# RMDLO/trackdlo

Measured on AMD Instinct MI355X. Metric: EM iterations/sec at N=50k cloud pts, M=50 nodes, higher is better.
Workload: dtype f32; 1 GPU; C2: 1 frame(s) per GPU, N=50000 points, M=50 nodes, 50 EM iterations per cpd_lle call, tol=0, trackdlo.launch parameters, fp32 E-step + fp64 M-step; whole calls (prune + sort + setup + loop + read-back), sorted-cloud reuse OFF, calls alternate between 2 resident (cloud, Y0) pairs; frames_per_gpu=1, parallelism=frames sharded, 1 rank(s), no data-path collective

## Files before the change

trackdlo_amd/csrc/tdlo_api.cpp:

```cpp
#include "../../include/trackdlo_hip.h"
#include "tdlo_internal.h"
#include "tdlo_host.h"
#include "tdlo_image.h"
#include "tdlo_rccl.h"

#include <algorithm>
#include <limits>
#include <chrono>
#include <cmath>
#include <cstdio>
#include <cstdlib>
#include <cstring>
#include <condition_variable>
#include <functional>
#include <mutex>
#include <string>
#include <thread>
#include <vector>

using namespace tdlo;

namespace {

#define TDLO_RET(x) do { hipError_t e_ = (x); if (e_ != hipSuccess) return e_; } while (0)
// ... 68 lines not shown
    }
    void loop(int idx) {
        (void)hipSetDevice(device);
        int seen = 0;
        for (;;) {
            std::function<int(int)> f;
            {
                std::unique_lock<std::mutex> lk(m);
                cv.wait(lk, [&] { return stop || gen != seen; });
                if (stop) return;
                seen = gen; f = job;
            }
            const int rc = f(idx);
            {
                std::lock_guard<std::mutex> lk(m);
                if (rc && !first_err) first_err = rc;
                if (--pending == 0) cv_done.notify_one();
            }
        }
    }
    int run(const std::function<int(int)> &f) {
        {
            std::lock_guard<std::mutex> lk(m);
            job = f; pending = (int)th.size(); first_err = 0; ++gen;
        }
        cv.notify_all();
        const int rc0 = f(0);
        std::unique_lock<std::mutex> lk(m);
        cv_done.wait(lk, [&] { return pending == 0; });
        return rc0 ? rc0 : first_err;
    }
    ~EnqueuePool() {
        { std::lock_guard<std::mutex> lk(m); stop = true; }
        cv.notify_all();
        for (auto &t : th) t.join();
    }
};

struct tdlo_ctx {
    int device = 0;
    hipStream_t stream = nullptr;
    double *xfer = nullptr;
    size_t xfer_doubles = 0;
    hipStream_t stream2[kBatchStreams - 1] = {};
    hipEvent_t evx[kBatchStreams] = {}, evj[kBatchStreams] = {};
    hipEvent_t ev[6] = {nullptr, nullptr, nullptr, nullptr, nullptr, nullptr};
    tdlo_config cfg{};
    std::vector<Slot> slots;
    std::vector<FrameDev> fh;
    FrameDev *fd = nullptr;
    double *pin = nullptr;
    double *reg_ws = nullptr;
    size_t reg_ws_cap = 0;
    void *cloud_ws = nullptr;
    size_t cloud_ws_cap = 0;
    void *cloud_fws = nullptr;
    size_t cloud_fws_cap = 0;
    bool cloud_fused_first = true;
    unsigned long long *cloud_res = nullptr;
    unsigned cloud_epoch = 0;
    char *img_pin = nullptr;
    size_t img_pin_cap = 0;
    int img_pin_rows = 0, img_pin_cols = 0;
    bool cloud_fused_on = !(getenv("TDLO_CLOUD_FUSED") && atoi(getenv("TDLO_CLOUD_FUSED")) == 0);
    bool cloud_team_on = !(getenv("TDLO_CLOUD_TEAM") && atoi(getenv("TDLO_CLOUD_TEAM")) == 0);
    unsigned long long *vis_state = nullptr, *vis_res = nullptr;
    unsigned vis_epoch = 0;
    bool vis_armed = false;
    double *vis_nodes_pin = nullptr;
    long long cloud_vis_rides = 0;
    long long vis_route[2] = {0, 0};
    long long cloud_route[2] = {0, 0};
    char *col_pin = nullptr;
    size_t col_pin_cap = 0;
    int col_pin_rows = 0, col_pin_cols = 0;
    void *col_dev = nullptr;
    size_t col_dev_cap = 0;
    bool colour_fused_on = !(getenv("TDLO_COLOUR_FUSED") && atoi(getenv("TDLO_COLOUR_FUSED")) == 0);
    long long colour_route[2] = {0, 0};
    const unsigned char *last_colour = nullptr, *last_occluder = nullptr;
    const void *view_img[4] = {nullptr, nullptr, nullptr, nullptr};
    int view_rows = 0, view_cols = 0;
    int last_col_rows = 0, last_col_cols = 0;
    char *res_pin = nullptr;
    size_t res_pin_cap = 0;
    int res_pin_rows = 0, res_pin_cols = 0;
    void *res_dev = nullptr;
    size_t res_dev_cap = 0;
    char *rnd_pin = nullptr, *rnd_dev = nullptr;
    bool render_inplace = !(getenv("TDLO_RENDER_INPLACE") && atoi(getenv("TDLO_RENDER_INPLACE")) == 0);
    long long render_route[2] = {0, 0};
    size_t pin_doubles = 0;
    std::string err;
    int last_F = 0;
    bool lle_batch_dense = false;
    bool lle_dense_once = false;
    long long band_retries = 0;
    long long route_count[6] = {0, 0, 0, 0, 0, 0};
    bool fuse_on = true;
    int fuse_force_timeout = getenv("TDLO_FUSE_FORCE_TIMEOUT") ? atoi(getenv("TDLO_FUSE_FORCE_TIMEOUT")) : 0;
    bool sort_reuse = !(getenv("TDLO_REUSE_SORT") && atoi(getenv("TDLO_REUSE_SORT")) == 0);
    double *mbox = nullptr;
    size_t mbox_doubles = 0;
    unsigned mbox_epoch = 0;
    bool direct_in = !(getenv("TDLO_DIRECT_UPLOAD") && atoi(getenv("TDLO_DIRECT_UPLOAD")) == 0);
    double *late_buf = nullptr;
    size_t late_doubles = 0;
    bool late_on = !(getenv("TDLO_LATE_PRIORS") && atoi(getenv("TDLO_LATE_PRIORS")) == 0);
    bool mbox_on = !(getenv("TDLO_HOST_MAILBOX") && atoi(getenv("TDLO_HOST_MAILBOX")) == 0);
    struct PairNext {
        int state = 0;
        int slot = 0, M = 0, n_vis = 0;
        double sigma2 = 0;
        tdlo_params p{};
        std::vector<double> Y;
        FrameDev f{};
        size_t up = 0;
        bool has_sums = false;
        bool ahead = false;
        bool cloud_in_pin = false;
        int spec = 0;
        unsigned spec_epoch = 0;
    } pair;
    double *pin2 = nullptr;
    size_t pin2_doubles = 0;
    bool pair_on = !(getenv("TDLO_PAIR_SETUP") && atoi(getenv("TDLO_PAIR_SETUP")) == 0);
    Slot twin;
    bool twin_busy = false;
    bool ahead_on = !(getenv("TDLO_AHEAD") && atoi(getenv("TDLO_AHEAD")) == 0);
    double *cloud_pin = nullptr;
    size_t cloud_pin_doubles = 0;
    int cloud_pending = -1;
    bool cloud_direct_on = !(getenv("TDLO_DIRECT_CLOUD") && atoi(getenv("TDLO_DIRECT_CLOUD")) == 0);
    bool view_inplace = !(getenv("TDLO_VIEW_INPLACE") && atoi(getenv("TDLO_VIEW_INPLACE")) == 0);
    long long view_route[2] = {0, 0};
    long long voxel_view_calls = 0;
    hipEvent_t ev_view = nullptr;
    int iter_hint = 0, iter_hint_next = 0;
    bool iter_hint_on = !(getenv("TDLO_ITER_HINT") && atoi(getenv("TDLO_ITER_HINT")) == 0);
    bool lle_next_on = !(getenv("TDLO_LLE_NEXT") && atoi(getenv("TDLO_LLE_NEXT")) == 0);
    bool spec_force_timeout = getenv("TDLO_SPEC_FORCE_TIMEOUT") && atoi(getenv("TDLO_SPEC_FORCE_TIMEOUT")) != 0;
    bool spec_on = !(getenv("TDLO_SPEC_MSTEP") && atoi(getenv("TDLO_SPEC_MSTEP")) == 0);
    bool pair_sums_on = !(getenv("TDLO_PAIR_SUMS") && atoi(getenv("TDLO_PAIR_SUMS")) == 0);
    int estep2_mode = getenv("TDLO_ESTEP2") ? atoi(getenv("TDLO_ESTEP2")) : -1;
    int estep2_rows = (getenv("TDLO_ESTEP2_ROWS") && atoi(getenv("TDLO_ESTEP2_ROWS")) == 16) ? 16 : 8;
    int estep2_blocks = getenv("TDLO_ESTEP2_BLOCKS") ? atoi(getenv("TDLO_ESTEP2_BLOCKS")) : 0;
    bool xch_self = getenv("TDLO_XCH_SELF") && atoi(getenv("TDLO_XCH_SELF")) != 0;
    bool boost_off_once = false;
    long long boost_retries = 0;
    bool test_boost_fail = getenv("TDLO_TEST_BOOST_FAIL") && atoi(getenv("TDLO_TEST_BOOST_FAIL")) != 0;
    int estep_wide_min = getenv("TDLO_ESTEP_WIDE") ? (atoi(getenv("TDLO_ESTEP_WIDE")) > 0 ? atoi(getenv("TDLO_ESTEP_WIDE")) : (1 << 30)) : kEstepWideMin;
    int fused_iter_mode = getenv("TDLO_FUSED_ITER") ? (atoi(getenv("TDLO_FUSED_ITER")) != 0 ? 1 : 0) : -1;
    long long fused_calls = 0;
    long long estep2_frames = 0;
    bool timing = false;
    EnqueuePool *pool = nullptr;
    int split_active = 0;
    double *xch_dmin = nullptr;
    double *xch_sums = nullptr;
    double *split_buf = nullptr;
    size_t split_buf_doubles = 0;
    void *own_comm = nullptr;
    unsigned long long *xch_own = nullptr;
    size_t xch_own_words = 0;
    int xch_rank = 0, xch_nranks = 0, xch_mcap = 0, xch_cap_ranks = 0;
    unsigned long long *xch_peer[kMaxXchRanks] = {};
    std::vector<void *> xch_opened;
    unsigned xch_calls = 0;
};

namespace {

struct HostProf {
    static constexpr int kN = 16;
    const char *name[kN] = {"set_cloud call", "guide nodes", "prepare_frame #1", "enqueue prologue #1", "enqueue iteration #1", "wait #1", "results #1",
                            "traverse + priors", "prepare_frame #2", "enqueue prologue #2", "enqueue iteration #2", "wait #2", "results #2", "between registrations", "", ""};
    double us[kN] = {};
    long n[kN] = {};
    bool on = getenv("TDLO_TRACK_PROFILE") && atoi(getenv("TDLO_TRACK_PROFILE")) != 0;
    int base = 0;
    std::chrono::steady_clock::time_point t0;
    void start() { if (on) t0 = std::chrono::steady_clock::now(); }
    void mark(int id) {
        if (!on) return;
        const auto t1 = std::chrono::steady_clock::now();
        us[id] += std::chrono::duration<double, std::micro>(t1 - t0).count(); ++n[id];
        t0 = t1;
    }
    void report() {
        if (!on) return;
        double tot = 0;
        for (int i = 0; i < kN; ++i) if (n[i]) tot += us[i] / (double)n[i];
        fprintf(stderr, "trackdlo_hip host profile (us per call of the phase; sum %.1f):\n", tot);
        for (int i = 0; i < kN; ++i) if (n[i]) fprintf(stderr, "  %-24s %8.2f  x %ld\n", name[i], us[i] / (double)n[i], n[i]);
    }
};
HostProf g_prof;

int fail(tdlo_ctx *c, int code, const std::string &msg) {
    if (c) c->err = msg;
    if (code == TDLO_E_HIP) (void)hipGetLastError();
    return code;
}

#define HIPCHK(c, call)                                                                        \
    do {                                                                                       \
        hipError_t e_ = (call);                                                                \
        if (e_ != hipSuccess)                                                                  \
            return fail((c), TDLO_E_HIP, std::string(#call) + ": " + hipGetErrorString(e_));   \
    } while (0)

hipError_t wait_stream(hipStream_t s) {
    static const int spin_us = getenv("TDLO_SPIN_US") ? atoi(getenv("TDLO_SPIN_US")) : 0;
    if (spin_us > 0) {
        const auto t0 = std::chrono::steady_clock::now();
        for (;;) {
            const hipError_t e = hipStreamQuery(s);
            if (e != hipErrorNotReady) return e;
            if (std::chrono::duration<double, std::micro>(std::chrono::steady_clock::now() - t0).count() > spin_us) break;
        }
    }
    return hipStreamSynchronize(s);
}

hipError_t drain_for_realloc(tdlo_ctx *c) {
    const hipError_t e = hipStreamSynchronize(c->stream);
    if (e != hipSuccess) return e;
    if (c->stream2[0]) return hipStreamSynchronize(c->stream2[0]);
    return hipSuccess;
}

enum class Staging {
    Pinned,
    PinnedZeroed,
    DeviceZeroed
};
static int grow_staging(tdlo_ctx *c, double *&buf, size_t &have, size_t doubles, Staging kind) {
    if (doubles <= have) return 0;
    const bool dev = kind == Staging::DeviceZeroed;
    HIPCHK(c, dev ? hipStreamSynchronize(c->stream) : drain_for_realloc(c));
    if (buf) { if (dev) hipFree(buf); else hipHostFree(buf); }
    buf = nullptr; have = 0;
    if (dev) {
        HIPCHK(c, hipMalloc((void **)&buf, doubles * sizeof(double)));
        HIPCHK(c, hipMemsetAsync(buf, 0, doubles * sizeof(double), c->stream));
    } else {
        HIPCHK(c, hipHostMalloc((void **)&buf, doubles * sizeof(double), hipHostMallocDefault));
        if (kind == Staging::PinnedZeroed) std::memset(buf, 0, doubles * sizeof(double));
    }
    have = doubles;
    return 0;
}
int ensure_pin(tdlo_ctx *c, size_t doubles) { return grow_staging(c, c->pin, c->pin_doubles, doubles, Staging::Pinned); }
int ensure_pin2(tdlo_ctx *c, size_t doubles) { return grow_staging(c, c->pin2, c->pin2_doubles, doubles, Staging::Pinned); }
int ensure_late(tdlo_ctx *c, size_t doubles) { return grow_staging(c, c->late_buf, c->late_doubles, doubles, Staging::PinnedZeroed); }
int ensure_mbox(tdlo_ctx *c, size_t doubles) { return grow_staging(c, c->mbox, c->mbox_doubles, doubles, Staging::PinnedZeroed); }
int ensure_cloud_pin(tdlo_ctx *c, size_t doubles) {
    if (doubles <= c->cloud_pin_doubles) return 0;
    return grow_staging(c, c->cloud_pin, c->cloud_pin_doubles, (doubles + 4095) & ~(size_t)4095, Staging::Pinned);
}
int ensure_xfer(tdlo_ctx *c, size_t doubles) { return grow_staging(c, c->xfer, c->xfer_doubles, doubles, Staging::DeviceZeroed); }

int mbox_wait(tdlo_ctx *c, hipStream_t stream, unsigned epoch, int min_it, bool need_done, unsigned long long *word) {
    const unsigned long long *w = (const unsigned long long *)(c->mbox + c->mbox_doubles - 2);
    auto t_chk = std::chrono::steady_clock::now();
    for (unsigned spins = 1;; ++spins) {
        const unsigned long long v = __atomic_load_n(w, __ATOMIC_ACQUIRE);
        if ((unsigned)(v >> 32) == epoch) {
            const bool done = (v >> 31) & 1u;
            if (done || (!need_done && (int)(v & 0x7fffffffu) >= min_it)) { *word = v; return 0; }
        }
        if ((spins & 255u) == 0) {
            const auto now = std::chrono::steady_clock::now();
            if (std::chrono::duration<double, std::micro>(now - t_chk).count() > 500.0) {
                t_chk = now;
                const hipError_t e = hipStreamQuery(stream);
                if (e == hipSuccess) {
                    const unsigned long long v2 = __atomic_load_n(w, __ATOMIC_ACQUIRE);
                    if ((unsigned)(v2 >> 32) == epoch && (((v2 >> 31) & 1u) || (!need_done && (int)(v2 & 0x7fffffffu) >= min_it))) { *word = v2; return 0; }
                    return 1;
                }
                if (e != hipErrorNotReady) return fail(c, TDLO_E_HIP, std::string("stream: ") + hipGetErrorString(e));
            }
        }
#if defined(__x86_64__)
        __builtin_ia32_pause();
#endif
    }
}

int ensure_points(tdlo_ctx *c, Slot &s, int n) {
    if (n <= s.cap_points) return 0;
    HIPCHK(c, drain_for_realloc(c));
    if (s.Xraw) hipFree(s.Xraw);
    if (s.Xs) hipFree(s.Xs);
    if (s.bucket) hipFree(s.bucket);
    if (s.blksum) hipFree(s.blksum);
    s.Xraw = nullptr; s.Xs = nullptr; s.bucket = nullptr; s.blksum = nullptr;
    s.cap_points = 0; s.N0 = 0;
    const size_t cap = ((size_t)n + 1023) & ~(size_t)1023;
    const size_t nb = cap / kBlock + 1;
    HIPCHK(c, hipMalloc((void **)&s.Xraw, 3 * cap * sizeof(double)));
    HIPCHK(c, hipMalloc((void **)&s.Xs, 3 * cap * sizeof(double)));
    HIPCHK(c, hipMalloc((void **)&s.bucket, cap * sizeof(unsigned short)));
    HIPCHK(c, hipMalloc((void **)&s.blksum, (nb + 2) * sizeof(double)));
    s.cap_points = (int)cap;
// ... 258 lines not shown
            HIPCHK(c, hipMalloc((void **)&s.hist, 2 * need * sizeof(int)));
            s.hist_ints = need;
        }
    }
    f.Xraw = s.Xraw; f.Xs = s.Xs; f.bucket = s.bucket; f.hist = s.hist; f.hist_off = s.hist + (size_t)f.nprune_blocks * M; f.blksum = s.blksum;
    f.keep = s.blksum + (size_t)s.cap_points / kBlock + 1;
    f.reuse_sorted = (c->sort_reuse && s.sorted_valid && s.sorted_prec == p->precision && s.sorted_Y.size() == 3 * (size_t)M &&
                      std::memcmp(s.sorted_Y.data(), Y, sizeof(double) * 3 * M) == 0) ? 1 : 0;
    f.Yin = blk + nc.Yin; f.ctr = blk + nc.ctr; f.Y = blk + nc.Y; f.Y0 = blk + nc.Y0; f.nodes = blk + nc.nodes;
    f.coord = blk + nc.coord; f.G = blk + nc.G; f.chain = blk + nc.chain; f.H = blk + nc.H; f.Hb = blk + nc.Hb; f.HG = blk + nc.HG; f.HY0 = blk + nc.HY0;
    f.aJ = blk + nc.aJ; f.aYd = blk + nc.aYd; f.dminbits = (unsigned long long *)(blk + nc.dmin);
    f.acc = (long long *)(blk + nc.acc);
    f.band = blk + nc.band;
    {
        int ln = 0; while (((long long)1 << ln) < (long long)s.N0 + 1) ++ln;
        double len = 0;
        for (int i = 0; i + 1 < M; ++i) { double d2 = 0; for (int d = 0; d < 3; ++d) { const double e = Y[d * M + i + 1] - Y[d * M + i]; d2 += e * e; } len += std::sqrt(d2); }
        int ld = 0; while (std::ldexp(1.0, ld) < 2.0 * (len + 0.2) && ld < 20) ++ld;
        static const int sh_coarser = getenv("TDLO_ACC_COARSER") ? atoi(getenv("TDLO_ACC_COARSER")) : 0;
        const int shP = std::min(60 - ln, 44) - sh_coarser;
        f.acc_sh[0] = shP; f.acc_sh[1] = shP - ld; f.acc_sh[2] = shP - 2 * ld;
        {
            static const int only = getenv("TDLO_ACC_COARSER_ONLY") ? atoi(getenv("TDLO_ACC_COARSER_ONLY")) : -1;
            if (only >= 0) for (int k = 0; k < 3; ++k) if (k != only) f.acc_sh[k] += sh_coarser;
        }
        const int lshare = std::min(51, 67 - std::max(ln, 6)), lpoint = std::min(51, 61 - ln);
        f.acc_lim[0] = std::ldexp(1.0, lshare - f.acc_sh[0]); f.acc_lim[1] = std::ldexp(1.0, lshare - f.acc_sh[1]); f.acc_lim[2] = std::ldexp(1.0, lpoint - f.acc_sh[2]);
    }
    f.acc_boost_off = c->boost_off_once ? 1 : (c->test_boost_fail ? -1 : 0);
    f.estep_wide_min = c->estep_wide_min;
    if (estep2_eligible(c, f) && (c->estep2_mode == 1 || nbatch >= kEstep2MinWaves)) estep2_geometry(c, f, false);
    choose_acc_rows(c, f, false);
    f.sums = blk + nc.sums; f.Ascr = blk + nc.Ascr; f.Yout = blk + nc.Yout; f.dbg = (unsigned long long *)(blk + nc.dbg);
    f.sync = s.sync;
    f.st = (IterState *)(blk + nc.st);
    if (hb_resident) f.Hb = s.hb_next;
    return 0;
}

hipError_t zero_accumulators(const std::vector<FrameDev> &fh, int F, hipStream_t s) {
    for (int i = 0; i < F; ++i) {
        const hipError_t e = hipMemsetAsync(fh[i].acc, 0, sizeof(long long) * 2 * kAccRows * (4 * (size_t)fh[i].M + 2), s);
        if (e != hipSuccess) return e;
    }
    return hipSuccess;
}

size_t upload_doubles(const NodeCarve &nc, const tdlo_params *p, bool band) { return p->include_lle ? (band ? nc.H : nc.upload) : nc.Hb; }

void fill_stats(tdlo_stats *st, const IterState &is) {
    st->iters = is.it; st->converged = is.converged; st->n_kept = is.N; st->status = is.status; st->sigma2 = is.sigma2;
    st->mstep_retries = is.retries;
}

typedef std::function<int(const double *&, int &)> LatePriors;

static unsigned next_mbox_epoch(tdlo_ctx *c) {
    unsigned e = ++c->mbox_epoch;
    if (e == 0) e = ++c->mbox_epoch;
    return e;
}

static FrameDev spec_mstep_descriptor(tdlo_ctx *c, const tdlo_ctx::PairNext &pn, unsigned epoch, const IterState *spec_prev, double *lle_next) {
    FrameDev fs = pn.f;
    fs.reuse_sorted = 1; fs.has_priors = 1;
    fs.late_aJ = c->late_buf; fs.late_aYd = c->late_buf + pn.M;
    fs.host_out = c->mbox; fs.host_prog = (unsigned long long *)(c->mbox + c->mbox_doubles - 2); fs.host_epoch = epoch;
    fs.host_report_it = (pn.p.tol <= 0.0 || pn.p.max_iter <= 2 * kChunkIters) ? 0 : std::max(1, std::min(std::min(c->iter_hint_next, kIterHintMax), pn.p.max_iter));
    fs.spec_flag = spec_flag_word(c); fs.spec_prev = spec_prev; fs.spec_epoch = epoch;
    if (lle_next) fs.lle_next = lle_next;
    return fs;
}

static int launch_ahead(tdlo_ctx *c) {
    tdlo_ctx::PairNext &pn = c->pair;
    const int M = pn.M;
    const int N0 = c->slots[pn.slot].N0;
    const NodeCarve nc(M);
    if (!pn.cloud_in_pin || N0 <= 0 || pn.p.include_lle || pn.p.max_iter <= 0 || M > kChainLdsMaxNodes) return 0;
    if (c->late_doubles < 4 * (size_t)M + 2 || c->mbox_doubles < nc.readback + 4 || c->cloud_pin_doubles < 3 * (size_t)N0) return 0;
    if (!c->stream2[0]) HIPCHK(c, hipStreamCreateWithFlags(&c->stream2[0], hipStreamNonBlocking));
    hipStream_t sb = c->stream2[0];
    Slot &tw = c->twin;
    const size_t need_hist = (size_t)((N0 + kBlock - 1) / kBlock) * M;
    const bool grow = N0 > tw.cap_points || M > tw.cap_nodes || need_hist > tw.hist_ints || nc.upload + 2 > c->pin2_doubles;
    if (grow || c->twin_busy) HIPCHK(c, hipStreamSynchronize(sb));
    c->twin_busy = false;
    int rc;
    if ((rc = ensure_points(c, tw, N0))) return rc;
    tw.N0 = N0; tw.sorted_valid = false;
    if ((rc = ensure_pin2(c, nc.upload + 2))) return rc;
    FrameDev &f = pn.f;
    if ((rc = prepare_frame(c, -1, pn.Y.data(), M, pn.sigma2, &pn.p, nullptr, 0, nullptr, pn.n_vis, nullptr, c->pin2, f, false))) return rc;
    if (grow) HIPCHK(c, hipStreamSynchronize(c->stream));
    if (!f.wide_tile || f.mstep_dense || f.reuse_sorted || !c->fuse_on || !prologue_pair_ok(f)) return 0;
    pn.up = upload_doubles(nc, &pn.p, false);
    f.Xhost = c->cloud_pin;
    std::memcpy(c->pin2 + nc.fdev, &f, sizeof(FrameDev));
    const unsigned fep = next_fuse_epoch(c, tw);
    c->twin_busy = true;
    HIPCHK(c, launch_prologue_direct(&f, c->pin2, tw.nodeblk, (int)pn.up, (int)nc.Yin, fep, sb));
    f.Xhost = nullptr;
    f.late_mstep = 1;
    const FrameDev *fdb = (const FrameDev *)(tw.nodeblk + nc.fdev);
    if (f.vis_branch) HIPCHK(c, launch_estep_only(fdb, &f, 1, 1, sb));
    HIPCHK(c, launch_estep_only(fdb, &f, 1, 0, sb));
    const unsigned e2 = next_mbox_epoch(c);
    const FrameDev fs = spec_mstep_descriptor(c, pn, e2, nullptr, nullptr);
    HIPCHK(c, launch_mstep_chain(fdb, &fs, 1, 0, fs.precision == TDLO_PREC_F64, sb));
    pn.has_sums = false; pn.spec = 1; pn.spec_epoch = e2; pn.ahead = true; pn.state = 2;
    return 0;
}

static int chunk_iters(int chunk, int left) { return std::min(chunk < 2 ? 1 : (chunk == 2 ? 2 : kChunkIters), left); }

static IterState readback_state(const double *blocks, size_t stride, const NodeCarve &nc, int i) {
    IterState is;
    std::memcpy(&is, blocks + (size_t)i * stride + (nc.st - nc.Yout), sizeof is);
    return is;
}
static bool every_frame_done(const double *blocks, size_t stride, const NodeCarve &nc, int F) {
    for (int i = 0; i < F; ++i) if (readback_state(blocks, stride, nc, i).done == 0) return false;
    return true;
}
static bool any_frame_ended_with(int status, const double *blocks, size_t stride, const NodeCarve &nc, int F) {
    for (int i = 0; i < F; ++i) if (readback_state(blocks, stride, nc, i).status == status) return true;
    return false;
}

int run_frames(tdlo_ctx *c, int F, const int *slots, double *Y, int M, double *sigma2, const tdlo_params *p,
               const double *priors, int K, const int *vis, int n_vis, const double *H_override, tdlo_stats *stats,
               const LatePriors *late = nullptr);

struct SpecGuard {
    tdlo_ctx *c; unsigned epoch = 0; bool live = false;
    void release(bool go) { if (live) { spec_release(c, epoch, go); live = false; } }
    ~SpecGuard() { release(false); }
};

struct FramesCall {
    tdlo_ctx *const c; const int F; const int *const slots; double *const Y; const int M; double *const sigma2; const tdlo_params *const p;
    const double *const priors; const int K; const int *const vis; const int n_vis; const double *const H_override; tdlo_stats *const stats;
    const LatePriors *const late;
    const int iter_hint;
    const bool timing;
    const NodeCarve nc;
    const bool merged;
    size_t up, ustride;
    const size_t fdd;
    bool paired = false;
    bool ahead = false;
    bool use_mbox = false;
    bool fused_mode = false;
    bool late_async = false;
    bool lle_next = false;
    hipStream_t s = nullptr;
    hipStream_t gs[kBatchStreams] = {};
    int goff[kBatchStreams + 1] = {};
    int NS = 1;
    bool forked = false;
    int enqueued = 0;
    bool sums_first = false;
    bool ahead_first = false;
    bool spec_released = false;
    unsigned epoch = 0;
    bool have_readback = false;
    const FrameDev *fdp = nullptr;
    double *nodeblk_used = nullptr;
    SpecGuard sg;

    FramesCall(tdlo_ctx *c_, int F_, const int *slots_, double *Y_, int M_, double *sigma2_, const tdlo_params *p_, const double *priors_, int K_,
               const int *vis_, int n_vis_, const double *H_override_, tdlo_stats *stats_, const LatePriors *late_, int iter_hint_)
        : c(c_), F(F_), slots(slots_), Y(Y_), M(M_), sigma2(sigma2_), p(p_), priors(priors_), K(K_), vis(vis_), n_vis(n_vis_), H_override(H_override_),
          stats(stats_), late(late_), iter_hint(iter_hint_), timing(c_->timing), nc(M_), merged(F_ > 1),
          up(upload_doubles(nc, p_, p_->include_lle && mstep_band_enabled() && !c_->lle_dense_once)), ustride(merged ? up : nc.upload),
          fdd(((size_t)F_ * sizeof(FrameDev) + 15) / 16 * 2), sg{c_} {}

    Slot &slot0() const { return c->slots[slots[0]]; }
    size_t rstride() const { return merged ? nc.readback : nc.upload; }
    bool fixed_count() const { return p->tol <= 0.0 || p->max_iter <= 2 * kChunkIters; }

    int size_staging();
    void recognise_pair();
    int stage_frames();
    int choose_batch_kernels();
    int choose_routes();
    int open_mailbox();
    int upload_and_prologue();
    int stage_late_priors();
    int fork_streams();
    void choose_loop();
    int drive_fixed();
    int drive_mailbox();
    int drive_polled();
    int read_back();
    bool repeat(int *rc);
    int results_out(std::chrono::steady_clock::time_point t_host0);

    FrameDev fused_copy(int k) const;
    hipError_t iterate(int n);
    hipError_t join();
    int mbox_done(int min_it, bool need_done, bool *done);
    int take_mbox(bool events_recorded);
    int launch_paired_mstep_ahead();
};

int FramesCall::size_staging() {
    int rc = ensure_pin(c, (size_t)F * std::max(nc.upload, nc.readback + 2) + fdd + 2 * (size_t)F * std::max(nc.readback, (sizeof(IterState) + 7) / 8) + 4);
    if (rc) return rc;
    if (merged) rc = ensure_xfer(c, (size_t)F * (upload_doubles(nc, p, false) + nc.readback) + fdd);
    return rc;
}

void FramesCall::recognise_pair() {
    if (late && c->pair.state == 2) {
        const tdlo_ctx::PairNext &pn = c->pair;
        const Slot &sl = slot0();
        const bool same = F == 1 && !priors && !H_override && pn.slot == slots[0] && pn.M == M && pn.n_vis == n_vis && pn.sigma2 == sigma2[0] && same_params(pn.p, *p) &&
                          std::memcmp(pn.Y.data(), Y, sizeof(double) * 3 * M) == 0 && pn.f.wide_tile != 0;
        if (pn.ahead) paired = ahead = same && c->stream2[0] != nullptr;
        else paired = same && sl.sorted_valid && sl.sorted_prec == p->precision &&
                      sl.sorted_Y.size() == 3 * (size_t)M && std::memcmp(sl.sorted_Y.data(), Y, sizeof(double) * 3 * M) == 0;
        c->pair.state = 0; c->pair.ahead = false;
    }
    if (late && c->pair.spec) { sg.epoch = c->pair.spec_epoch; sg.live = true; c->pair.spec = 0; }
    if (!paired) sg.release(false);
    c->fh.assign(F, FrameDev{});
    if (paired) {
        c->fh[0] = c->pair.f; c->fh[0].reuse_sorted = 1; up = c->pair.up;
        if (ahead) ++c->route_count[4];
        else { ++c->route_count[0]; if (c->pair.has_sums) ++c->route_count[1]; }
    }
}

int FramesCall::stage_frames() {
    for (int pass = 0; pass < 2 && !paired; ++pass) {
        for (int i = 0; i < F; ++i) {
            const int rc = prepare_frame(c, slots[i], Y + (size_t)i * 3 * M, M, sigma2[i], p, priors, K, vis, n_vis, H_override,
                                         c->pin + (size_t)i * ustride, c->fh[i], false, !merged);
            if (rc) return rc;
            if (merged) {
                FrameDev &f = c->fh[i];
                f.wide_tile = 0;
                if (c->cfg.estep_blocks <= 0 && f.nblkE >= 64) f.nblkE = (f.nblkE + 1) / 2;
                double *bu = c->xfer + (size_t)i * up, *br = c->xfer + (size_t)F * up + fdd + (size_t)i * nc.readback;
                f.Yin = bu + nc.Yin; f.aJ = bu + nc.aJ; f.aYd = bu + nc.aYd;
                if (p->include_lle) { f.Hb = bu + nc.Hb; f.H = bu + nc.H; }
                f.Yout = br; f.st = (IterState *)(br + (nc.st - nc.Yout));
            }
        }
        if (merged) { const int rc = choose_batch_kernels(); if (rc) return rc; }
        if (!p->include_lle) break;
        bool all_band = true;
        for (int i = 0; i < F; ++i) all_band = all_band && c->fh[i].lle_band;
        if (all_band) break;
        if (!merged) { up = upload_doubles(nc, p, false); break; }
        if (pass == 0) { c->lle_batch_dense = true; up = upload_doubles(nc, p, false); ustride = up; }
    }
    c->lle_batch_dense = false;
    return 0;
}

int FramesCall::choose_batch_kernels() {
    long long waves = 0;
    bool elig = true;
    for (int i = 0; i < F; ++i) { waves += (c->fh[i].N0 + 63) / 64; elig = elig && estep2_eligible(c, c->fh[i]); }
    const bool two = elig && (c->estep2_mode == 1 || waves >= kEstep2MinWaves);
    for (int i = 0; i < F; ++i) if (two) estep2_geometry(c, c->fh[i], true);
    for (int i = 0; i < F; ++i) choose_acc_rows(c, c->fh[i], true);
    {
        static const int env = getenv("TDLO_ACC_ROWS") ? atoi(getenv("TDLO_ACC_ROWS")) : 0;
        bool small = env == 0 && !p->include_lle;
        for (int i = 0; i < F; ++i) small = small && c->fh[i].nblkE <= 64 && !c->fh[i].mstep_dense && c->fh[i].M <= kChunk;
        if (small) for (int i = 0; i < F; ++i) c->fh[i].acc_rows = 2;
    }
    if (!two) for (int i = 0; i < F; ++i) if (c->fh[i].estep2) return fail(c, TDLO_E_INVALID, "internal: a batch's frames disagree about the E-step kernel");
    return 0;
}

int FramesCall::choose_routes() {
    if (!merged && !paired && p->include_lle && c->fh[0].lle_band && slot0().hb_next != nullptr && c->fh[0].Hb == slot0().hb_next)
        { up = nc.Hb; ++c->route_count[3]; }
    lle_next = late != nullptr && !merged && !ahead && c->lle_next_on && !p->include_lle && !c->fh[0].mstep_dense && M <= 256 && p->max_iter > 0 &&
               slot0().hb_next_cap >= M;
    if (lle_next) { c->fh[0].lle_next = slot0().hb_next; slot0().hb_next_valid = false; }
    late_async = late != nullptr && c->fh[0].wide_tile != 0 && (c->late_on || paired);
    if (late && !late_async) {
        const double *lp = nullptr; int lk = 0;
        int rc;
        if ((rc = (*late)(lp, lk))) return rc;
        if ((rc = stage_priors(c, c->pin + nc.aJ, c->pin + nc.aYd, Y, M, lp, lk, p->alpha))) return rc;
        c->fh[0].has_priors = lk > 0 ? 1 : 0;
    }
    g_prof.mark(g_prof.base + 2);
    {
        bool all_reuse = true;
        for (int i = 0; i < F; ++i) all_reuse = all_reuse && c->fh[i].reuse_sorted;
        if (!all_reuse) for (int i = 0; i < F; ++i) c->fh[i].reuse_sorted = 0;
    }
    return 0;
}

int FramesCall::open_mailbox() {
    use_mbox = !merged && c->mbox_on && p->max_iter > 0 &&
               ((!p->include_lle && !c->fh[0].mstep_dense) || (p->include_lle && c->fh[0].lle_band));
    if (!use_mbox) { sg.release(false); return 0; }
    const int rc = ensure_mbox(c, nc.readback + 4);
    if (rc) return rc;
    epoch = sg.live ? sg.epoch : next_mbox_epoch(c);
    c->fh[0].host_out = c->mbox; c->fh[0].host_prog = (unsigned long long *)(c->mbox + c->mbox_doubles - 2); c->fh[0].host_epoch = epoch;
    return 0;
}

int FramesCall::upload_and_prologue() {
    int rc;
    s = ahead ? c->stream2[0] : c->stream;
    if (timing) HIPCHK(c, hipEventRecord(c->ev[0], s));
    if (merged) {
        std::memcpy(c->pin + (size_t)F * up, c->fh.data(), sizeof(FrameDev) * F);
        HIPCHK(c, hipMemcpyAsync(c->xfer, c->pin, ((size_t)F * up + fdd) * sizeof(double), hipMemcpyHostToDevice, s));
        fdp = (const FrameDev *)(c->xfer + (size_t)F * up);
    } else {
        if (!paired) std::memcpy(c->pin + nc.fdev, c->fh.data(), sizeof(FrameDev));
        nodeblk_used = ahead ? c->twin.nodeblk : (paired ? slot0().nodeblk2 : slot0().nodeblk);
        fdp = (const FrameDev *)(nodeblk_used + nc.fdev);
    }
    if (c->cloud_pending >= 0) {
        const bool fused = !merged && !paired && c->direct_in && c->fuse_on && c->cloud_pending == slots[0] && !c->fh[0].reuse_sorted && prologue_pair_ok(c->fh[0]);
        if (fused) { c->fh[0].Xhost = c->cloud_pin; c->cloud_pending = -1; }
        else if ((rc = flush_pending_cloud(c))) return rc;
    }
    if (paired) {
    } else if (!merged && c->direct_in && (c->fuse_on || c->fh[0].reuse_sorted) && prologue_direct_ok(c->fh[0])) {
        Slot &sl = slot0();
        const unsigned fep = c->fh[0].reuse_sorted ? 0u : next_fuse_epoch(c, sl);
        tdlo_ctx::PairNext &pn = c->pair;
        const FrameDev *f2 = nullptr;
        if (pn.state == 1) {
            pn.state = 0;
            if (!late && !c->fh[0].reuse_sorted && prologue_pair_ok(c->fh[0]) && pn.slot == slots[0] && pn.M == M && !pn.p.include_lle) {
                const NodeCarve nc2(pn.M);
                if ((rc = ensure_pin2(c, nc2.upload + 2))) return rc;
                if ((rc = prepare_frame(c, pn.slot, pn.Y.data(), pn.M, pn.sigma2, &pn.p, nullptr, 0, nullptr, pn.n_vis, nullptr, c->pin2, pn.f, true))) return rc;
                if (pn.f.wide_tile && !pn.f.mstep_dense && !pn.f.vis_branch) {
                    pn.up = upload_doubles(nc2, &pn.p, false);
                    std::memcpy(c->pin2 + nc2.fdev, &pn.f, sizeof(FrameDev));
                    f2 = &pn.f;
                    pn.has_sums = p->include_lle && c->fh[0].lle_band && !c->fh[0].vis_branch && p->mu == pn.p.mu && p->precision == pn.p.precision &&
                                  sigma2[0] == pn.sigma2 && std::memcmp(Y, pn.Y.data(), sizeof(double) * 3 * M) == 0 && p->max_iter > 0 && c->pair_sums_on;
                    if (pn.has_sums) c->fh[0].pair_sums = sl.nodeblk2 + nc2.sums;
                }
            }
        }
        HIPCHK(c, launch_prologue_direct(c->fh.data(), c->pin, sl.nodeblk, (int)up, (int)nc.Yin, fep, s, f2, c->pin2, sl.nodeblk2, f2 ? (int)pn.up : 0));
        c->fh[0].Xhost = nullptr;
        if (f2) pn.state = 2;
    } else {
        if (!merged) HIPCHK(c, hipMemcpyAsync(slot0().nodeblk, c->pin, up * sizeof(double), hipMemcpyHostToDevice, s));
        HIPCHK(c, launch_prune_and_setup(fdp, c->fh.data(), F, s));
    }
    g_prof.mark(g_prof.base + 3);
    for (int i = 0; i < F; ++i) {
        Slot &sl = c->slots[slots[i]];
        if (!c->fh[i].reuse_sorted) { sl.sorted_Y.assign(Y + (size_t)i * 3 * M, Y + (size_t)(i + 1) * 3 * M); sl.sorted_prec = p->precision; sl.sorted_valid = true; }
    }
    return 0;
}

int FramesCall::stage_late_priors() {
    if (late_async) {
        const double *lp = nullptr; int lk = 0;
        int rc = (*late)(lp, lk);
        if (!rc) rc = ensure_late(c, 4 * (size_t)M);
        if (!rc) rc = stage_priors(c, c->late_buf, c->late_buf + M, Y, M, lp, lk, p->alpha);
        if (rc) { sg.release(false); (void)hipStreamSynchronize(s); return rc; }
        if (lk <= 0) sg.release(false);
        c->fh[0].has_priors = lk > 0 ? 1 : 0;
        c->fh[0].late_aJ = c->late_buf; c->fh[0].late_aYd = c->late_buf + M;
        g_prof.mark(7);
    }
    if (timing) HIPCHK(c, hipEventRecord(c->ev[1], s));
    return 0;
}

int FramesCall::fork_streams() {
    static const int ns_env = getenv("TDLO_BATCH_STREAMS") ? atoi(getenv("TDLO_BATCH_STREAMS")) : 0;
    NS = ns_env > 0 ? ns_env : (F >= 28 ? 3 : (F >= 16 ? 4 : (F >= 8 ? 2 : 1)));
    NS = std::max(1, std::min(std::min(NS, kBatchStreams), F));
    for (int g = 0; g <= NS; ++g) goff[g] = (int)(((long long)F * g) / NS);
    gs[0] = s;
    for (int g = 1; g < NS; ++g) {
        if (!c->stream2[g - 1]) HIPCHK(c, hipStreamCreateWithFlags(&c->stream2[g - 1], hipStreamNonBlocking));
        gs[g] = c->stream2[g - 1];
    }
    return 0;
}

void FramesCall::choose_loop() {
    sums_first = paired && !ahead && c->pair.has_sums;
    ahead_first = ahead;
    fused_mode = !merged && F == 1 && !paired && !ahead && late == nullptr && c->pair.state == 0 && use_mbox && !sums_first && !ahead_first &&
                 fused_iter_eligible(c, c->fh[0]);
    if (fused_mode) ++c->fused_calls;
}

FrameDev FramesCall::fused_copy(int k) const {
    FrameDev fc = c->fh[0];
    if (k & 1) { double *blk = nodeblk_used; fc.Yout = blk + nc.Yout2; fc.st = (IterState *)(blk + nc.st2); fc.Y = blk + nc.Y2; fc.nodes = blk + nc.nodes2; }
    return fc;
}

hipError_t FramesCall::iterate(int n) {
    for (int it = 0; it < n; ++it) {
        ++enqueued;
        if (fused_mode) {
            const int k = enqueued - 1;
            if (k == 0) TDLO_RET(launch_estep_only(fdp, c->fh.data(), 1, 0, s));
            if (k + 1 < p->max_iter) TDLO_RET(launch_iter_fused(fused_copy(k), fused_copy(k + 1), k, s));
            else TDLO_RET(launch_mstep_chain_close(fused_copy(k), k, s));
            continue;
        }
        if (sums_first || ahead_first) {
            const bool from_given = sums_first;
            sums_first = false; ahead_first = false;
            if (sg.live) { sg.release(!c->spec_force_timeout); spec_released = true; if (!ahead) ++c->route_count[2]; }
            else if (from_given) TDLO_RET(launch_mstep_chain(fdp, c->fh.data(), 1, 1, c->fh[0].precision == TDLO_PREC_F64, s));
            else {
                c->fh[0].late_mstep = 0;
                TDLO_RET(launch_iteration(fdp, c->fh.data(), 1, s));
            }
            c->fh[0].late_mstep = 0;
            continue;
        }
        for (int g = 0; g < NS; ++g) {
            const FrameDev *fdg = fdp + goff[g], *fhg = c->fh.data() + goff[g];
            const int Fg = goff[g + 1] - goff[g];
            if (NS > 1 && !forked && g + 1 < NS) {
                if (fhg[0].vis_branch) TDLO_RET(launch_estep_only(fdg, fhg, Fg, 1, gs[g]));
                TDLO_RET(launch_estep_only(fdg, fhg, Fg, 0, gs[g]));
                TDLO_RET(hipEventRecord(c->evx[g], gs[g]));
                TDLO_RET(hipStreamWaitEvent(gs[g + 1], c->evx[g], 0));
                TDLO_RET(launch_estep_only(fdg, fhg, Fg, 2, gs[g]));
            } else {
                TDLO_RET(launch_iteration(fdg, fhg, Fg, gs[g], enqueued - 1));
            }
        }
        forked = true;
    }
    return hipSuccess;
}

hipError_t FramesCall::join() {
    if (NS < 2 || !forked) return hipSuccess;
    for (int g = 1; g < NS; ++g) {
        TDLO_RET(hipEventRecord(c->evj[g - 1], gs[g]));
        TDLO_RET(hipStreamWaitEvent(s, c->evj[g - 1], 0));
    }
    return hipSuccess;
}

int FramesCall::mbox_done(int min_it, bool need_done, bool *done) {
    unsigned long long w = 0;
    int wr = mbox_wait(c, s, epoch, min_it, need_done, &w);
    if (wr == 1 && spec_released) {
        spec_released = false;
        IterState is;
        HIPCHK(c, hipMemcpy(&is, c->fh[0].st, sizeof is, hipMemcpyDeviceToHost));
        int have = is.it;
        if (!ahead && !is.done && have == 0 && enqueued > 0) { HIPCHK(c, launch_mstep_chain(fdp, c->fh.data(), 1, 1, c->fh[0].precision == TDLO_PREC_F64, s)); have = 1; }
        for (; !is.done && have < enqueued; ++have) HIPCHK(c, launch_iteration(fdp, c->fh.data(), 1, s));
        wr = mbox_wait(c, s, epoch, min_it, need_done, &w);
    }
    if (wr < 0) return wr;
    if (wr == 1) return fail(c, TDLO_E_HIP, "the stream drained, but the M-step did not report the state of the registration");
    *done = (w >> 31) & 1u;
    return 0;
}

int FramesCall::take_mbox(bool events_recorded) {
    std::memcpy(c->pin, c->mbox, nc.readback * sizeof(double));
    have_readback = true;
    if (timing) {
        if (!events_recorded) { HIPCHK(c, hipEventRecord(c->ev[2], s)); HIPCHK(c, hipEventRecord(c->ev[3], s)); }
        HIPCHK(c, hipEventSynchronize(c->ev[3]));
    }
    return 0;
}

int FramesCall::drive_fixed() {
    static const bool pool_on = !(getenv("TDLO_BATCH_THREADS") && atoi(getenv("TDLO_BATCH_THREADS")) == 0);
    int rc;
    if (NS > 1 && pool_on && p->max_iter >= 8) {
        HIPCHK(c, iterate(1));
        if (!c->pool) { c->pool = new EnqueuePool; c->pool->start(kBatchStreams - 1, c->device); }
        const int rest = p->max_iter - 1;
        const int prc = c->pool->run([&](int g) -> int {
            if (g >= NS) return 0;
            const FrameDev *fdg = fdp + goff[g], *fhg = c->fh.data() + goff[g];
            const int Fg = goff[g + 1] - goff[g];
            for (int it = 0; it < rest; ++it) { const hipError_t e = launch_iteration(fdg, fhg, Fg, gs[g], 1 + it); if (e != hipSuccess) return (int)e; }
            return 0;
        });
        if (prc) return fail(c, TDLO_E_HIP, std::string("batch enqueue: ") + hipGetErrorString((hipError_t)prc));
    } else {
        HIPCHK(c, iterate(p->max_iter));
    }
    if (use_mbox) {
        if (timing) { HIPCHK(c, hipEventRecord(c->ev[2], s)); HIPCHK(c, hipEventRecord(c->ev[3], s)); }
        bool done = false;
        if ((rc = mbox_done(0, true, &done))) return rc;
        if ((rc = take_mbox(true))) return rc;
    }
    return 0;
}

int FramesCall::launch_paired_mstep_ahead() {
    tdlo_ctx::PairNext &pn = c->pair;
    Slot &sl = slot0();
    const NodeCarve nc2(pn.M);
    const int rc = ensure_late(c, 4 * (size_t)pn.M + 2);
    if (rc) return rc;
    const unsigned e2 = next_mbox_epoch(c);
    const bool leaves_lle = c->lle_next_on && pn.M <= 256 && sl.hb_next_cap >= pn.M;
    const FrameDev fs = spec_mstep_descriptor(c, pn, e2, c->fh[0].st, leaves_lle ? sl.hb_next : nullptr);
    HIPCHK(c, launch_mstep_chain((const FrameDev *)(sl.nodeblk2 + nc2.fdev), &fs, 1, 1, fs.precision == TDLO_PREC_F64, s));
    pn.spec = 1; pn.spec_epoch = e2;
    return 0;
}

int FramesCall::drive_mailbox() {
    int rc;
    const int first = std::max(1, std::min(std::min(iter_hint, kIterHintMax), p->max_iter));
    c->fh[0].host_report_it = first;
    HIPCHK(c, iterate(first));
    if (!late && c->pair.state == 2 && c->pair.has_sums && c->spec_on && c->mbox_on && !timing && c->pair.p.max_iter > 0) {
        if ((rc = launch_paired_mstep_ahead())) return rc;
    } else if (!late && c->pair.state == 3) {
        c->pair.state = 0; c->pair.ahead = false;
        if (c->spec_on && c->mbox_on && !timing && c->pair.slot == slots[0] && (rc = launch_ahead(c))) { spec_abort(c); return rc; }
    }
    g_prof.mark(g_prof.base + 4);
    bool stop = false;
    if ((rc = mbox_done(first, false, &stop))) { spec_abort(c); return rc; }
    if (!stop && !c->pair.ahead) c->pair.spec = 0;
    g_prof.mark(g_prof.base + 5);
    int launched = first;
    for (int chunk = 0; launched < p->max_iter && !stop; ++chunk) {
        const int n = chunk_iters(chunk, p->max_iter - launched);
        c->fh[0].host_report_it = launched + n;
        HIPCHK(c, iterate(n));
        launched += n;
        if ((rc = mbox_done(launched - n, false, &stop))) return rc;
    }
    if (!stop && (rc = mbox_done(0, true, &stop))) return rc;
    return take_mbox(false);
}

int FramesCall::drive_polled() {
    IterState *flags = (IterState *)(c->pin + (size_t)F * nc.upload + fdd);
    double *fl_rb = c->pin + (size_t)F * nc.upload + fdd;
    const double *results_dev = merged ? c->xfer + (size_t)F * up + fdd : nodeblk_used + nc.Yout;
    HIPCHK(c, iterate(1));
    HIPCHK(c, join());
    if (timing) HIPCHK(c, hipEventRecord(c->ev[2], s));
    HIPCHK(c, hipMemcpyAsync(c->pin, results_dev, (size_t)F * nc.readback * sizeof(double), hipMemcpyDeviceToHost, s));
    if (timing) HIPCHK(c, hipEventRecord(c->ev[3], s));
    HIPCHK(c, wait_stream(s));
    have_readback = every_frame_done(c->pin, rstride(), nc, F);
    int launched = 1;
    bool stop = have_readback;
    for (int chunk = 0; launched < p->max_iter && !stop; ++chunk) {
// ... 1750 lines not shown
        double tot = 0;
        for (int r = -3; r < reps; ++r) {
            if (fh[0].vis_branch) HIPCHK(c, launch_estep_only(c->fd, fh.data(), F, 1, s));
            HIPCHK(c, launch_estep_only(c->fd, fh.data(), F, 0, s));
            if (kind == 4) HIPCHK(c, launch_estep_only(c->fd, fh.data(), F, 3, s));
            if (r >= 0) HIPCHK(c, hipEventRecord(evs[2 * r], s));
            HIPCHK(c, launch_estep_only(c->fd, fh.data(), F, kind, s));
            if (r >= 0) HIPCHK(c, hipEventRecord(evs[2 * r + 1], s));
            if (kind == 3) HIPCHK(c, launch_estep_only(c->fd, fh.data(), F, 4, s));
        }
        HIPCHK(c, hipStreamSynchronize(s));
        for (int r = 0; r < reps; ++r) { float ms = 0; hipEventElapsedTime(&ms, evs[2 * r], evs[2 * r + 1]); tot += ms; }
        for (auto &e : evs) hipEventDestroy(e);
        if (avg_us) *avg_us = (float)(tot * 1000.0 / reps);
    } else {
    for (int w = 0; w < 3; ++w) HIPCHK(c, launch_estep_only(c->fd, fh.data(), F, kind, s));
    HIPCHK(c, hipEventRecord(c->ev[0], s));
    for (int r = 0; r < reps; ++r) HIPCHK(c, launch_estep_only(c->fd, fh.data(), F, kind, s));
    HIPCHK(c, hipEventRecord(c->ev[1], s));
    HIPCHK(c, hipStreamSynchronize(s));
    float ms = 0;
    hipEventElapsedTime(&ms, c->ev[0], c->ev[1]);
    if (avg_us) *avg_us = ms * 1000.0f / (float)reps;
    }
    }
    HIPCHK(c, zero_accumulators(fh, F, s));
    for (int i = 0; i < F; ++i) {
        std::memcpy(c->pin + i * 16, &saved[i], sizeof(IterState));
        HIPCHK(c, hipMemcpyAsync(c->fh[i].st, c->pin + i * 16, sizeof(IterState), hipMemcpyHostToDevice, s));
    }
    HIPCHK(c, hipMemcpyAsync(c->fd, c->fh.data(), sizeof(FrameDev) * F, hipMemcpyHostToDevice, s));
    HIPCHK(c, hipStreamSynchronize(s));
    return TDLO_OK;
}

int tdlo_profile_iteration(tdlo_ctx *c, int reps, float *estep_us, float *mstep_us, float *iter_us, char *mstep_kernel, int name_cap) {
    if (!c || c->last_F < 1 || c->fh.empty()) return TDLO_E_INVALID;
    if (reps < 1 || reps > 256) return fail(c, TDLO_E_INVALID, "bad reps");
    HIPCHK(c, hipSetDevice(c->device));
    hipStream_t s = c->stream;
    const int F = c->last_F;
    std::vector<IterState> saved(F);
    for (int i = 0; i < F; ++i) HIPCHK(c, hipMemcpyAsync(&saved[i], c->fh[i].st, sizeof(IterState), hipMemcpyDeviceToHost, s));
    HIPCHK(c, hipStreamSynchronize(s));
    for (int i = 0; i < F; ++i) {
        IterState is = saved[i];
        is.done = 0; is.it = 0;
        std::memcpy(c->pin + i * 16, &is, sizeof is);
        HIPCHK(c, hipMemcpyAsync(c->fh[i].st, c->pin + i * 16, sizeof(IterState), hipMemcpyHostToDevice, s));
    }
    std::vector<FrameDev> fh = c->fh;
    for (auto &f : fh) { f.max_iter = 1 << 30; f.tol = -1.0; }
    HIPCHK(c, hipMemcpyAsync(c->fd, fh.data(), sizeof(FrameDev) * F, hipMemcpyHostToDevice, s));
    HIPCHK(c, zero_accumulators(fh, F, s));
    std::vector<hipEvent_t> evs(4 * (size_t)reps, nullptr);
    for (auto &e : evs) HIPCHK(c, hipEventCreate(&e));
    for (int w = 0; w < 3; ++w) HIPCHK(c, launch_iteration(c->fd, fh.data(), F, s, w));
    HIPCHK(c, hipEventRecord(c->ev[0], s));
    for (int r = 0; r < reps; ++r) HIPCHK(c, launch_iteration_timed(c->fd, fh.data(), F, s, evs[4 * r], evs[4 * r + 1], evs[4 * r + 2], evs[4 * r + 3], 3 + r));
    HIPCHK(c, hipEventRecord(c->ev[1], s));
    HIPCHK(c, hipStreamSynchronize(s));
    double te = 0, tm = 0;
    bool m_ok = true;
    for (int r = 0; r < reps; ++r) {
        float ms = 0;
        hipEventElapsedTime(&ms, evs[4 * r], evs[4 * r + 1]); te += ms;
        if (hipEventElapsedTime(&ms, evs[4 * r + 2], evs[4 * r + 3]) == hipSuccess) tm += ms; else m_ok = false;
    }
    (void)hipGetLastError();
    float tot = 0;
    hipEventElapsedTime(&tot, c->ev[0], c->ev[1]);
    for (auto &e : evs) hipEventDestroy(e);
    if (estep_us) *estep_us = (float)(te * 1000.0 / reps);
    if (mstep_us) *mstep_us = m_ok ? (float)(tm * 1000.0 / reps) : -1.0f;
    if (iter_us) *iter_us = tot * 1000.0f / (float)reps;
    if (mstep_kernel && name_cap > 0) { std::strncpy(mstep_kernel, mstep_kernel_name(fh.data(), F), (size_t)name_cap - 1); mstep_kernel[name_cap - 1] = 0; }
    for (int i = 0; i < F; ++i) {
        std::memcpy(c->pin + i * 16, &saved[i], sizeof(IterState));
        HIPCHK(c, hipMemcpyAsync(c->fh[i].st, c->pin + i * 16, sizeof(IterState), hipMemcpyHostToDevice, s));
    }
    HIPCHK(c, zero_accumulators(fh, F, s));
    HIPCHK(c, hipMemcpyAsync(c->fd, c->fh.data(), sizeof(FrameDev) * F, hipMemcpyHostToDevice, s));
    HIPCHK(c, hipStreamSynchronize(s));
    return TDLO_OK;
}

int tdlo_debug_read_cloud(tdlo_ctx *c, int frame, double *out, int max_points, double *ctr) {
    if (!c || frame < 0 || frame >= (int)c->fh.size() || !out) return TDLO_E_INVALID;
    const FrameDev &f = c->fh[frame];
    IterState is;
    HIPCHK(c, hipMemcpy(&is, f.st, sizeof is, hipMemcpyDeviceToHost));
    const int N = is.N;
    if (N > max_points) return TDLO_E_INVALID;
    const size_t es = f.precision == TDLO_PREC_F64 ? 8 : 4;
    std::vector<char> buf(es * (size_t)N);
    for (int d = 0; d < 3; ++d) {
        HIPCHK(c, hipMemcpy(buf.data(), (const char *)f.Xs + es * (size_t)f.ldx * d, es * (size_t)N, hipMemcpyDeviceToHost));
        for (int n = 0; n < N; ++n) out[(size_t)d * N + n] = es == 8 ? ((const double *)buf.data())[n] : (double)((const float *)buf.data())[n];
    }
    if (ctr) HIPCHK(c, hipMemcpy(ctr, f.ctr, 3 * sizeof(double), hipMemcpyDeviceToHost));
    return N;
}

int tdlo_debug_read_setup(tdlo_ctx *c, int frame, int what, double *out, int cap) {
    if (!c || frame < 0 || frame >= (int)c->fh.size() || !out) return TDLO_E_INVALID;
    const FrameDev &f = c->fh[frame];
    const int M = f.M;
    HIPCHK(c, hipStreamSynchronize(c->stream));
    const double *src = nullptr;
    int n = 0;
    switch (what) {
    case TDLO_SETUP_COORD: src = f.coord; n = M; break;
    case TDLO_SETUP_CHAIN: src = f.chain; n = 8 * M; break;
    case TDLO_SETUP_HY0: src = f.include_lle ? f.HY0 : nullptr; n = 3 * M; break;
    case TDLO_SETUP_Y0: src = f.Y0; n = 3 * M; break;
    case TDLO_SETUP_NODES: {
        n = 4 * M;
        if (n > cap || !f.nodes) return TDLO_E_INVALID;
        if (f.precision == TDLO_PREC_F64) { HIPCHK(c, hipMemcpy(out, f.nodes, sizeof(double) * n, hipMemcpyDeviceToHost)); return n; }
        std::vector<float> buf((size_t)n);
        HIPCHK(c, hipMemcpy(buf.data(), f.nodes, sizeof(float) * n, hipMemcpyDeviceToHost));
        for (int i = 0; i < n; ++i) out[i] = (double)buf[i];
        return n;
    }
    case TDLO_SETUP_KEEP: {
        n = 4;
        if (n > cap || !f.keep || !f.st) return TDLO_E_INVALID;
        IterState is;
        HIPCHK(c, hipMemcpy(out, f.keep, 2 * sizeof(double), hipMemcpyDeviceToHost));
        HIPCHK(c, hipMemcpy(&is, f.st, sizeof is, hipMemcpyDeviceToHost));
        out[2] = (double)is.N; out[3] = is.sum_d2;
        return n;
    }
    case TDLO_SETUP_SIGMA2: {
        n = 1;
        if (n > cap || !f.st) return TDLO_E_INVALID;
        IterState is;
        HIPCHK(c, hipMemcpy(&is, f.st, sizeof is, hipMemcpyDeviceToHost));
        out[0] = is.sigma2;
        return n;
    }
    default: return TDLO_E_INVALID;
    }
    if (!src || n > cap) return TDLO_E_INVALID;
    HIPCHK(c, hipMemcpy(out, src, sizeof(double) * n, hipMemcpyDeviceToHost));
    return n;
}

int tdlo_debug_mstep_dense(int on) { return mstep_set_dense(on); }
int tdlo_debug_mstep_lle_dense(int on) { return mstep_set_lle_dense(on); }
long long tdlo_debug_band_retries(tdlo_ctx *c) { return c ? c->band_retries : -1; }

long long tdlo_debug_route_count(tdlo_ctx *c, int which) {
    if (!c || which < 0 || which > 23) return -1;
    if (which >= 22) return c->vis_route[which - 22];
    if (which == 21) return c->voxel_view_calls;
    if (which >= 19) return c->render_route[which - 19];
    if (which >= 17) return c->view_route[which - 17];
    if (which >= 15) return c->colour_route[which - 15];
    if (which == 14) return c->fused_calls;
    if (which >= 11 && which <= 13) return 0;
    if (which == 10) return c->boost_retries;
    if (which == 9) return c->estep2_frames;
    if (which == 8) return c->cloud_vis_rides;
    return which < 6 ? c->route_count[which] : c->cloud_route[which - 6];
}

int tdlo_debug_lle_band_device(tdlo_ctx *c, const double *Y, int M, double *Hb) {
    if (!c) return TDLO_E_INVALID;
    if (!Y || !Hb || M < 1 || M > 256) return fail(c, TDLO_E_INVALID, "tdlo_debug_lle_band_device: 1 .. 256 nodes");
    HIPCHK(c, hipSetDevice(c->device));
    double *d = nullptr;
    HIPCHK(c, hipMalloc((void **)&d, sizeof(double) * 16 * (size_t)M));
    hipError_t e = hipMemcpyAsync(d, Y, sizeof(double) * 3 * M, hipMemcpyHostToDevice, c->stream);
    if (e == hipSuccess) e = launch_lle_band_debug(d, M, d + 3 * M, c->stream);
    if (e == hipSuccess) e = hipMemcpyAsync(Hb, d + 3 * M, sizeof(double) * 13 * M, hipMemcpyDeviceToHost, c->stream);
    if (e == hipSuccess) e = hipStreamSynchronize(c->stream);
    (void)hipFree(d);
    HIPCHK(c, e);
    return TDLO_OK;
}
int tdlo_debug_fail_hip(tdlo_ctx *c) {
    if (!c) return TDLO_E_INVALID;
    HIPCHK(c, hipSetDevice(c->device));
    HIPCHK(c, hipMemcpy(nullptr, nullptr, 16, hipMemcpyDeviceToDevice));
    return TDLO_OK;
}

int tdlo_pci_bus_id(tdlo_ctx *c, char *out, int len) {
    if (!c || !out || len < 16) return TDLO_E_INVALID;
    HIPCHK(c, hipDeviceGetPCIBusId(out, len, c->device));
    return TDLO_OK;
}

int tdlo_set_xch_self(tdlo_ctx *c, int on) {
    if (!c) return TDLO_E_INVALID;
    const int prev = c->xch_self ? 1 : 0;
    c->xch_self = on != 0;
    return prev;
}

int tdlo_set_sort_reuse(tdlo_ctx *c, int on) {
    if (!c) return TDLO_E_INVALID;
    const int prev = c->sort_reuse ? 1 : 0;
    c->sort_reuse = on != 0;
    return prev;
}

int tdlo_set_timing(tdlo_ctx *c, int on) {
    if (!c) return TDLO_E_INVALID;
    const int prev = c->timing ? 1 : 0;
    c->timing = on != 0;
    return prev;
}

int tdlo_debug_stamps(tdlo_ctx *c, int slot, unsigned long long *out, int n) {
    if (!c || slot < 0 || slot >= (int)c->slots.size() || !out || n < 1 || n > 64 || c->fh.empty()) return TDLO_E_INVALID;
    const int dbg_frame = getenv("TDLO_DEBUG_FRAME") ? atoi(getenv("TDLO_DEBUG_FRAME")) : 0;
    if (dbg_frame < 0 || dbg_frame >= (int)c->fh.size()) return TDLO_E_INVALID;
    HIPCHK(c, hipMemcpyAsync(c->pin, c->fh[dbg_frame].dbg, sizeof(unsigned long long) * n, hipMemcpyDeviceToHost, c->stream));
    HIPCHK(c, hipStreamSynchronize(c->stream));
    std::memcpy(out, c->pin, sizeof(unsigned long long) * n);
    return TDLO_OK;
}

int tdlo_debug_cloud_stamps(tdlo_ctx *c, unsigned long long *out, int n) {
    if (!c || !out || n < 0 || n > 24) return TDLO_E_INVALID;
    if (!c->cloud_fws) return fail(c, TDLO_E_INVALID, "no depth -> cloud call yet");
    HIPCHK(c, hipStreamSynchronize(c->stream));
    HIPCHK(c, hipMemcpy(out, (const char *)c->cloud_fws + 64, sizeof(unsigned long long) * n, hipMemcpyDeviceToHost));
    return TDLO_OK;
}

int tdlo_debug_exp2(tdlo_ctx *c, const double *x, double *y, int n) {
    if (!c || !x || !y || n < 1) return TDLO_E_INVALID;
    HIPCHK(c, hipSetDevice(c->device));
    double *d = nullptr;
    HIPCHK(c, hipMalloc((void **)&d, 2 * (size_t)n * sizeof(double)));
    hipError_t e = hipMemcpyAsync(d, x, (size_t)n * sizeof(double), hipMemcpyHostToDevice, c->stream);
    if (e == hipSuccess) e = launch_debug_exp2(d, d + n, n, c->stream);
    if (e == hipSuccess) e = hipMemcpyAsync(y, d + n, (size_t)n * sizeof(double), hipMemcpyDeviceToHost, c->stream);
    if (e == hipSuccess) e = hipStreamSynchronize(c->stream);
    hipFree(d);
    HIPCHK(c, e);
    return TDLO_OK;
}

int tdlo_calc_lle_weights(int k, const double *Y, int M, double *L) {
    if (!Y || !L || M < 1 || k < 2 || k > 13) return TDLO_E_INVALID;
    lle_weights(k, Y, M, L);
    return TDLO_OK;
}

int tdlo_calc_lle_regulariser(const double *Y, int M, double *H, double *Hb) {
    if (!Y || M < 1 || (!H && !Hb)) return TDLO_E_INVALID;
    if (H) {
        std::vector<double> L((size_t)M * M);
        lle_weights(6, Y, M, L.data());
        lle_regulariser(L.data(), M, H);
    }
    if (Hb) lle_regulariser_band(Y, M, Hb);
    return TDLO_OK;
}

int tdlo_line_sphere_intersection(const double A[3], const double B[3], const double C[3], double radius, double out[6]) {
    Vec3 o[2];
    const int n = line_sphere(Vec3{A[0], A[1], A[2]}, Vec3{B[0], B[1], B[2]}, Vec3{C[0], C[1], C[2]}, radius, o);
    for (int i = 0; i < n; ++i) { out[3 * i] = o[i].x; out[3 * i + 1] = o[i].y; out[3 * i + 2] = o[i].z; }
    return n;
}

double tdlo_piecewise_error(const double *Y_track, int n_track, const double *Y_true, int n_true) {
    if (!Y_track || !Y_true || n_track < 1 || n_true < 2) return -1.0;
    return piecewise_error(Y_track, n_track, Y_true, n_true);
}

double tdlo_compute_error(const double *Y_track, int n_track, const double *Y_true, int n_true) {
    if (!Y_track || !Y_true || n_track < 2 || n_true < 2) return -1.0;
    return 0.5 * (piecewise_error(Y_track, n_track, Y_true, n_true) + piecewise_error(Y_true, n_true, Y_track, n_track));
}

int tdlo_traverse_euclidean(const double *coord, int n_coord, const double *guide, int Mg, const int *vis, int n_vis,
                            int alignment, int anchor, double *out) {
    if (!coord || !guide || !vis || !out) return TDLO_E_INVALID;
    std::vector<double> cv(coord, coord + n_coord), res;
    std::vector<int> vv(vis, vis + n_vis);
    const int n = traverse_euclidean(cv, guide, Mg, vv, alignment, anchor, res);
    if (n < 0) return TDLO_E_TRAVERSE;
    std::memcpy(out, res.data(), sizeof(double) * res.size());
    return n;
}

}

struct tdlo_tracker {
    tdlo_ctx *ctx;
    int slot;
    int M;
    int precision = TDLO_PREC_F32;
    std::vector<double> Y;
    std::vector<double> guide_nodes;
    int Mg;
    double sigma2, beta, beta_pre_proc, lambda, lambda_pre_proc, alpha, k_vis, mu, tol, lle_weight;
    int max_iter;
    std::vector<double> geodesic_coord;
    std::vector<double> priors;
    double visibility_threshold;
// ... 406 lines not shown
```

trackdlo_amd/csrc/tdlo_estep_body.h:

```cpp
#pragma once
#include "tdlo_devcommon.h"
#include "tdlo_estep_wide.h"
#include "tdlo_mstep_generic.h"
#include <type_traits>

namespace tdlo {

template <typename T> struct EstepHand {
    T x, y, z;
    const IterState *st;
    int acc_buf;
    int err_w;
    int acc_rows;
};

template <typename T, int EB> static size_t estep_lds_bytes(int M, bool single) {
    const int rt = (M <= kChunk && single) ? kChunk : tile_rows<T>(M <= kChunk ? 1 : 2);
    const int rows = M < rt ? M : rt;
    constexpr int NWE = EB / 64;
    const size_t tile = sizeof(T) * (((size_t)NWE * rows * kPStride + 7) & ~(size_t)3);
    const size_t red = (size_t)NWE * 64 * 4 * sizeof(double);
    size_t b = sizeof(V4<T>) * (size_t)M + sizeof(V4<T>) * NWE * kPtsStride + sizeof(T) * (size_t)((M + 3) & ~3);
    b += (tile > red ? tile : red) + 16 * sizeof(double) + 64;
    b += sizeof(double) * (size_t)(M <= kChunk ? NWE : 1) * M * 4;
    return b;
}

}
```

trackdlo_amd/csrc/tdlo_estep_body.inc:

```
    constexpr int NWE = EB / 64;
#ifdef TDLO_ESTEP_STAMPS
    if (threadIdx.x == 0) atomicMin(&f.dbg[32], (unsigned long long)__builtin_amdgcn_s_memrealtime());
#endif
#ifdef TDLO_ESTEP_STAMPS
#define ESTAMP(i) do { if (threadIdx.x == 0 && blockIdx.x == 0) f.dbg[40 + (i)] = __builtin_amdgcn_s_memtime(); } while (0)
#else
#define ESTAMP(i) do { } while (0)
#endif
#ifdef TDLO_ESTEP_PHASES
    unsigned long long ph_prev = __builtin_amdgcn_s_memtime(), ph_acc[10] = {0, 0, 0, 0, 0, 0, 0, 0, 0, 0};
#define EPHASE(i) do { asm volatile("s_waitcnt vmcnt(0) lgkmcnt(0)" ::: "memory"); const unsigned long long t_ = __builtin_amdgcn_s_memtime(); ph_acc[i] += t_ - ph_prev; ph_prev = t_; } while (0)
#else
#define EPHASE(i) do { } while (0)
#endif
    ESTAMP(0);
    const auto stg = TDLO_AS_GLOBAL(IterState, f.st);
#ifdef TDLO_TIMELINE
    const int tl_it = stg->it - 20;
    if (threadIdx.x == 0 && blockIdx.x == 0 && tl_it >= 0 && tl_it < 8) f.dbg[4 * tl_it] = __builtin_amdgcn_s_memrealtime();
#endif
    const int M = f.M;
    const int tid = threadIdx.x, lane = tid & 63;
    const int wave = __builtin_amdgcn_readfirstlane(tid >> 6);
    constexpr int TR = tile_rows<T>(NCH);
    constexpr int RT = (NCH == 1 && SINGLE) ? kChunk : TR;
    constexpr int RS = (RT / TR) * TR;
    const int rows = M < RT ? M : RT;
    V4<T> *nodesL = (V4<T> *)smem;
    V4<T> *pts = nodesL + M;
    T *lvL = (T *)(pts + NWE * kPtsStride);
    T *pbase = lvL + ((M + 3) & ~3);
    T *pb = pbase + (size_t)wave * rows * kPStride;
    double *scratch = (double *)(pbase + (((size_t)NWE * rows * kPStride + 7) & ~(size_t)3));

    const auto nodes = TDLO_AS_CONST(V4<T>, f.nodes);
    const auto xs = TDLO_AS_GLOBAL(T, f.Xs);
    const size_t ld = f.ldx;
    const int batch0 = blockIdx.x * NWE + wave;
    T x = 0, y = 0, z = 0;
    if constexpr (FUSED) { x = hand->x; y = hand->y; z = hand->z; }
    else {
        const int n = batch0 * 64 + lane;
        if (n < f.N0) { x = xs[n]; y = xs[ld + n]; z = xs[2 * ld + n]; }
    }
    constexpr bool EARLY = sizeof(T) == 4;
    static_assert(!FUSED || (sizeof(T) == 4 && NCH == 1 && SINGLE && !VIS), "the one-launch iteration carries the fp32 E-step of one frame on up to 64 nodes");
    const int done = FUSED ? 0 : stg->done;
    const int it0 = FUSED ? 0 : (EARLY ? stg->it : 0);
    int N; T k2, cn;
    if constexpr (FUSED) { N = hand->st->N; k2 = (T)hand->st->k2; cn = (T)hand->st->c_norm; }
    else if constexpr (EARLY) { N = stg->N; k2 = (T)stg->k2; cn = (T)stg->c_norm; }
    const int shb_e = FUSED ? hand->st->sh_boost : (EARLY ? stg->sh_boost : 0);
    const double rwin_e = FUSED ? hand->st->rwin32 : (EARLY ? stg->rwin32 : 0.0);
    const int par_e = FUSED ? hand->acc_buf : (it0 & 1);
    const auto qg = TDLO_AS_GLOBAL(V4<T>, f.nodes);
    V4<T> nd0; nd0.x = 0; nd0.y = 0; nd0.z = 0; nd0.w = 0;
    if (!FUSED && EARLY && tid < M) { nd0.x = qg[tid].x; nd0.y = qg[tid].y; nd0.z = qg[tid].z; nd0.w = qg[tid].w; }
#ifdef TDLO_NO_LANE_NODES
    constexpr bool LANE_NODES = false;
#else
    constexpr bool LANE_NODES = SINGLE && NCH == 1;
#endif
    V4<T> qn; qn.x = 0; qn.y = 0; qn.z = 0; qn.w = 0;
    if constexpr (FUSED) { if (LANE_NODES && lane < M) qn = nodesL[lane]; }
    else
    if (LANE_NODES && lane < M) { qn.x = qg[lane].x; qn.y = qg[lane].y; qn.z = qg[lane].z; qn.w = qg[lane].w; }
    if (!FUSED && SINGLE && f.late_aJ != nullptr && f.late_mstep == 0 && blockIdx.x == 0 && (EARLY ? it0 : stg->it) == 0) {
        double *dj = (double *)f.aJ, *dy = (double *)f.aYd;
        for (int i = threadIdx.x; i < f.M; i += EB) dj[i] = f.late_aJ[i];
        for (int i = threadIdx.x; i < 3 * f.M; i += EB) dy[i] = f.late_aYd[i];
    }
    if constexpr (FUSED) {
    } else if constexpr (EARLY) {
        if (tid < M) nodesL[tid] = nd0;
        for (int m = tid + EB; m < M; m += EB) { V4<T> o; o.x = qg[m].x; o.y = qg[m].y; o.z = qg[m].z; o.w = qg[m].w; nodesL[m] = o; }
    } else {
        N = stg->N; k2 = (T)stg->k2; cn = (T)stg->c_norm;
        for (int m = tid; m < M; m += EB) { V4<T> o; o.x = qg[m].x; o.y = qg[m].y; o.z = qg[m].z; o.w = qg[m].w; nodesL[m] = o; }
    }
    auto lane_val = [&](T v, int src) -> T {
        if constexpr (sizeof(T) == 4) return __uint_as_float((unsigned)__builtin_amdgcn_readlane((int)__float_as_uint(v), src));
        else return __hiloint2double(__builtin_amdgcn_readlane(__double2hiint(v), src), __builtin_amdgcn_readlane(__double2loint(v), src));
    };
    if (done) return;
    double lv_span = 0;
    if (VIS) {
        double tot = 0, dmx = 0, dmn = 1e300;
        for (int m = tid; m < M; m += EB) {
            double d = ::sqrt(Num<T>::from_bits(f.dminbits[m]));
            if (d > 10000.0) d = 10000.0;
            if (d <= f.vis_thr) d = 0;
            tot += ::exp(-f.k_vis * d);
            dmx = d > dmx ? d : dmx; dmn = d < dmn ? d : dmn;
        }
        tot = block_sum_n<NWE>(tot, scratch);
        {
            dmx = wave_max_nonneg(dmx); dmn = wave_min_nonneg(dmn);
            __syncthreads();
            if (lane == 0) { scratch[wave] = dmx; scratch[NWE + wave] = dmn; }
            __syncthreads();
#pragma unroll
            for (int w_ = 0; w_ < NWE; ++w_) { dmx = scratch[w_] > dmx ? scratch[w_] : dmx; dmn = scratch[NWE + w_] < dmn ? scratch[NWE + w_] : dmn; }
            lv_span = f.k_vis * (dmx - dmn) * 1.4426950408889634;
            if (!(lv_span > 0)) lv_span = 0;
        }
        for (int m = tid; m < M; m += EB) {
            double d = ::sqrt(Num<T>::from_bits(f.dminbits[m]));
            if (d > 10000.0) d = 10000.0;
            if (d <= f.vis_thr) d = 0;
            lvL[m] = (T)(-f.k_vis * d * 1.4426950408889634 - ::log2(tot));
        }
    }
    __syncthreads();
    ESTAMP(1);
    EPHASE(0);

    long long accQ = 0;
    const int shb = EARLY ? shb_e : stg->sh_boost;
    const double scP = acc_scale(f.acc_sh[0]), scR = acc_scale(f.acc_sh[1] + shb), scQ = acc_scale(f.acc_sh[2] + 2 * shb);
    const double limP = f.acc_lim[0], limR = f.acc_lim[1] * acc_scale(-shb), limQ = f.acc_lim[2] * acc_scale(-2 * shb);
    const double limQn = acc_scale(51 - (f.acc_sh[2] + 2 * shb));
    bool acc_ok = true;
    long long *accL = (long long *)(scratch + 16) + (NCH == 1 ? (size_t)wave * M * 4 : (size_t)0);
    if (NCH == 1) {
        for (int i = lane; i < M * 4; i += 64) accL[i] = 0;
    } else {
        for (int i = tid; i < M * 4; i += EB) accL[i] = 0;
        __syncthreads();
    }
    const T R2win = (T)((EARLY ? rwin_e : stg->rwin64) * (1.0 + (VIS ? lv_span / (sizeof(T) == 4 ? f.win_e32 : f.win_e64) : 0.0)));

    const int nbatch = (N + 63) >> 6;
    for (int batch = batch0; batch < nbatch; batch += f.nblkE * NWE) {
        const int n = batch * 64 + lane;
        const bool valid = n < N;
        EPHASE(6);
        if (batch != batch0) { x = 0; y = 0; z = 0; if (valid) { x = xs[n]; y = xs[ld + n]; z = xs[2 * ld + n]; } }
        else if (!valid) { x = 0; y = 0; z = 0; }
        EPHASE(1);
        int plo = 0, phi = M - 1;
        {
            const T cx = bcast_first(x), cy = bcast_first(y), cz = bcast_first(z);
            T r2 = valid ? (x - cx) * (x - cx) + (y - cy) * (y - cy) + (z - cz) * (z - cz) : T(0);
            T Dm[NCH];
            T dmin_w = Num<T>::inf();
#pragma unroll
            for (int c = 0; c < NCH; ++c) {
                const int m = c * kChunk + lane;
                Dm[c] = Num<T>::inf();
                if (m < M) { const V4<T> qq = LANE_NODES ? qn : nodesL[m]; Dm[c] = (qq.x - cx) * (qq.x - cx) + (qq.y - cy) * (qq.y - cy) + (qq.z - cz) * (qq.z - cz); }
                dmin_w = tmin(dmin_w, Dm[c]);
            }
            wave_max_min_nonneg(r2, dmin_w, r2, dmin_w);
            T lim = (Num<T>::sqrt_fast(dmin_w) + T(2) * Num<T>::sqrt_fast(r2)) * T(1.0001) + T(1e-30);
            lim = lim * lim;
            int first = M, last = -1;
#pragma unroll
            for (int c = 0; c < NCH; ++c) {
                const unsigned long long cand = __ballot(c * kChunk + lane < M && Dm[c] <= lim);
                if (cand) {
                    const int lo_c = c * kChunk + (int)__builtin_ctzll(cand), hi_c = c * kChunk + 63 - (int)__builtin_clzll(cand);
                    first = lo_c < first ? lo_c : first; last = hi_c > last ? hi_c : last;
                }
            }
            if (last >= 0) { plo = first; phi = last; }
            plo = __builtin_amdgcn_readfirstlane(plo); phi = __builtin_amdgcn_readfirstlane(phi);
        }
        ESTAMP(8);
        T best = Num<T>::inf();
        int a = plo;
        if constexpr (LANE_NODES) {
            for (int m = plo; m <= phi; ++m) {
                const T dx = x - lane_val(qn.x, m), dy = y - lane_val(qn.y, m), dz = z - lane_val(qn.z, m);
                const T d2 = dx * dx + dy * dy + dz * dz;
                if (d2 < best) { best = d2; a = m; }
            }
        } else {
            int m0 = plo;
            for (; m0 + 3 <= phi; m0 += 4) {
                const Node4<T> q4 = load_node4<T>(f.nodes, m0);
#pragma unroll
                for (int k = 0; k < 4; ++k) {
                    const T dx = x - q4.v[4 * k], dy = y - q4.v[4 * k + 1], dz = z - q4.v[4 * k + 2];
                    const T d2 = dx * dx + dy * dy + dz * dz;
                    if (d2 < best) { best = d2; a = m0 + k; }
                }
            }
            if (m0 <= phi) {
                const Node4<T> q4 = load_node4<T>(f.nodes, m0);
#pragma unroll
                for (int k = 0; k < 4; ++k) {
                    if (m0 + k <= phi) {
                        const T dx = x - q4.v[4 * k], dy = y - q4.v[4 * k + 1], dz = z - q4.v[4 * k + 2];
                        const T d2 = dx * dx + dy * dy + dz * dz;
                        if (d2 < best) { best = d2; a = m0 + k; }
                    }
                }
            }
        }
        {
            const bool under = best * k2 < T(-1075);
            if (__builtin_expect(__ballot(under) != 0ull, 0)) {
                const V4<T> q0 = nodesL[0];
                const T dx0 = x - q0.x, dy0 = y - q0.y, dz0 = z - q0.z;
                const T d0 = dx0 * dx0 + dy0 * dy0 + dz0 * dz0;
                if (under) { a = 0; best = d0; }
            }
        }
        ESTAMP(2);
        EPHASE(2);
        const int c1 = (a == 0) ? 2 : a - 1;
        const int c2 = (a == M - 1) ? M - 3 : a + 1;
        const V4<T> q1 = nodesL[c1], q2 = nodesL[c2], qa = nodesL[a];
        T dx = x - q1.x, dy = y - q1.y, dz = z - q1.z;
        const T s1 = dx * dx + dy * dy + dz * dz;
        dx = x - q2.x; dy = y - q2.y; dz = z - q2.z;
        const T s2 = dx * dx + dy * dy + dz * dz;
        bool first; T eb;
        if constexpr (sizeof(T) == 4) { first = s1 < s2; eb = Num<T>::sqrt_fast(first ? s1 : s2); }
        else { const T e1 = Num<T>::sqrt_fast(s1), e2 = Num<T>::sqrt_fast(s2); first = e1 < e2; eb = first ? e1 : e2; }
        const int b = first ? c1 : c2;
        const T cb = first ? q1.w : q2.w;
        const T ea = Num<T>::sqrt_fast(best);
        const bool a_lo = a < b;
        const int lo = a_lo ? a : b, hi = a_lo ? b : a;
        const T d_lo = a_lo ? ea : eb, d_hi = a_lo ? eb : ea;
        const T c_lo = a_lo ? qa.w : cb, c_hi = a_lo ? cb : qa.w;

        int wlo = 0, whi = M - 1;
        int min_lo = 0, max_hi = M - 1;
        bool gap_any = true;
        {
            T amin, amax, bmx;
            if constexpr (sizeof(T) == 8) {
                const unsigned klo = valid ? (unsigned)(kMaxNodes - lo) : 0u, khi = valid ? (unsigned)hi : 0u, kgap = (valid && hi - lo != 1) ? 1u : 0u;
                const unsigned zz = rows_max_u32(fold16_max(fold32_max(klo, khi), fold32_max(kgap, kgap)));
                min_lo = kMaxNodes - __builtin_amdgcn_readlane((int)zz, 15); max_hi = __builtin_amdgcn_readlane((int)zz, 47);
                gap_any = __builtin_amdgcn_readlane((int)zz, 31) != 0;
                bmx = wave_max_nonneg(valid ? best : T(0));
                amin = nodesL[min_lo].w; amax = nodesL[max_hi].w;
            } else {
                wave_min_max_max_nonneg(valid ? c_lo : Num<T>::inf(), valid ? c_hi : T(0), valid ? best : T(0), amin, amax, bmx);
            }
            const T Rwin = Num<T>::sqrt_fast(bmx + R2win);
            int first = M, last = -1;
#pragma unroll
            for (int c = 0; c < NCH; ++c) {
                const int m = c * kChunk + lane;
                const T cm = (m < M) ? (LANE_NODES ? qn.w : nodesL[m].w) : Num<T>::inf();
                const unsigned long long inw = __ballot(m < M && cm > amin - Rwin && cm < amax + Rwin);
                if (inw) {
                    const int lo_c = c * kChunk + (int)__builtin_ctzll(inw), hi_c = c * kChunk + 63 - (int)__builtin_clzll(inw);
                    first = lo_c < first ? lo_c : first; last = hi_c > last ? hi_c : last;
                }
            }
            if (last >= 0) { wlo = first; whi = last; }
            wlo = __builtin_amdgcn_readfirstlane(wlo); whi = __builtin_amdgcn_readfirstlane(whi);
        }

        ESTAMP(3);
        EPHASE(3);
        const bool adj = sizeof(T) == 8 ? !gap_any : __ballot(valid && hi - lo != 1) == 0;
        if constexpr (sizeof(T) == 8 && NCH > 1) {
            constexpr int WCH = NCH < 5 ? NCH : 5;
            if (whi - wlo + 1 >= f.estep_wide_min && whi - wlo + 1 <= 64 * WCH) {
                estep_wide_batch<WCH, VIS>(lane, wlo, whi, batch * 64, N, adj, min_lo, max_hi, x, y, z, lo, hi, c_lo, d_lo, c_hi, d_hi, k2, cn, nodesL, lvL, (double *)pb, accL,
                                           scP, scR, scQ, limP, limR, limQ, limQn, accQ, acc_ok);
                EPHASE(5);
                continue;
            }
        }
        T sum = 0, qs = 0;
        auto geo64 = [&](int m, T cm) -> T {
            if (adj) {
                if (m <= min_lo) { const T t = (c_lo - cm) + d_lo; return t * t; }
                if (m >= max_hi) { const T t = (cm - c_hi) + d_hi; return t * t; }
                return geo_arg_adj<T>(m, lo, cm, c_lo, d_lo, c_hi, d_hi);
            }
// ... 182 lines not shown
```

trackdlo_amd/csrc/tdlo_internal.h:

```cpp
#pragma once
#include <hip/hip_runtime.h>
#include <stdint.h>

namespace tdlo {

constexpr int kBlock = 256;
constexpr int kWave = 64;
constexpr int kChunk = 64;
constexpr int kPStride = 65;
constexpr int kPtsStride = 68;
constexpr int kAccRows = 8;
constexpr int kTileRows = 24;
constexpr int kTileRows32 = 16;
#ifndef TDLO_TILE_ROWS_LONG
#define TDLO_TILE_ROWS_LONG 24
#endif
template <typename T> __host__ __device__ constexpr int tile_rows(int nch) { return nch == 1 ? (sizeof(T) == 4 ? kTileRows32 : kTileRows) : TDLO_TILE_ROWS_LONG; }
constexpr int kMaxNodes = 1024;
constexpr int kChainLdsMaxNodes = 512;
constexpr int kLdsSolveMaxM = 128;
constexpr int kMaxXchRanks = 8;
#define TDLO_E_FUSE (-100)

struct IterState {
    double sigma2;
    double k2;
    double c_norm;
    double crit;
    double Np;
    double sum_d2;
    double Nc;
    double rwin32, rwin64;
    int N;
    int it;
    int done;
    int converged;
    int status;
    int retry_pending;
    int retries;
    int sh_boost;
};

struct FrameDev {
    int N0, M, ldx, nblkE;
    int max_iter, include_lle, has_priors, vis_branch;
    int precision, nprune_blocks, eb, wide_tile;
    double tol, beta, lambda, lle_weight, mu, alpha, k_vis, vis_thr, sigma2_in;
    const double *Xraw;
    void *Xs;
    unsigned short *bucket;
    int *hist;
    int *hist_off;
    double *blksum;
    const double *Yin;
    double *ctr;
    double *Y;
    double *Y0;
    void *nodes;
    double *coord;
    double *G;
    double *chain;
    const double *H;
    const double *Hb;
    double *HG;
    double *HY0;
    const double *aJ;
    const double *aYd;
    unsigned long long *dminbits;
    long long *acc;
    int acc_sh[3];
    double acc_lim[3];
    int force_timeout_it;
    int prune_tiles;
    int reuse_sorted;
    double *keep;
    int need_G;
    int mstep_dense;
    int h_banded;
    int lle_band;
    double *band;
    double band_s2_max;
    double *sums;
    double *Ascr;
    double *Yout;
    unsigned long long *dbg;
    unsigned *sync;
    IterState *st;
    double win_e32, win_e64;
    const double *late_aJ, *late_aYd;
    double *host_out;
    unsigned long long *host_prog;
    unsigned host_epoch;
    int host_report_it;
    unsigned long long *xch_inbox[kMaxXchRanks];
    int xch_rank, xch_nranks, xch_mcap;
    int xch_self;
    unsigned xch_epoch;
    double *pair_sums;
    const unsigned long long *spec_flag;
    const IterState *spec_prev;
    unsigned spec_epoch;
    double *lle_next;
    const double *Xhost;
    int late_mstep;
    int estep2;
    int acc_boost_off;
    int estep_wide_min;
    int acc_rows;
};
constexpr int kFusedErrWord = 112;

__host__ __device__ inline size_t xch_off_flag_init(int R) { (void)R; return 0; }
__host__ __device__ inline size_t xch_off_flag_dmin(int R) { return (size_t)R; }
__host__ __device__ inline size_t xch_off_flag_sums(int R) { return 3 * (size_t)R; }
__host__ __device__ inline size_t xch_off_init(int R) { return (5 * (size_t)R + 7) & ~(size_t)7; }
__host__ __device__ inline size_t xch_off_dmin(int R, int Mc) { (void)Mc; return xch_off_init(R) + 2 * (size_t)R; }
__host__ __device__ inline size_t xch_off_sums(int R, int Mc) { return xch_off_dmin(R, Mc) + 2 * (size_t)R * Mc; }
__host__ __device__ inline size_t xch_words(int R, int Mc) { return xch_off_sums(R, Mc) + 2 * (size_t)R * (4 * (size_t)Mc + 2); }

constexpr int kBandSlots = 13;
constexpr size_t kBandLdsLimit = 160 * 1024 - 1024;
struct BandPlan {
    int nU, tw, cT, cB, D, mT, mB, nUp, limT, sT, sB, nRecT, nRecB;
    __host__ __device__ explicit BandPlan(int M, int allow_twisted = 1) {
        nU = 2 * M;
        tw = (allow_twisted && nU >= 38) ? 1 : 0;
        for (;;) {
            if (!tw) { cT = (nU + kBandSlots - 1) / kBandSlots; cB = 0; D = 0; }
            else { const int q = nU - 12, ch = (q + kBandSlots - 1) / kBandSlots; D = kBandSlots * ch - q; cT = (ch + 1) / 2; cB = ch - cT; }
            mT = kBandSlots * cT; mB = kBandSlots * cB; nUp = nU + D;
            limT = tw ? mT + 12 : nU;
            sT = kBandSlots * (cT + tw); sB = tw ? kBandSlots * (cB + 1) : 0;
            nRecT = sT + 15; nRecB = tw ? sB + 15 : 0;
            if (!tw || lds_doubles(M) * 8 <= kBandLdsLimit) break;
            tw = 0;
        }
    }
    __host__ __device__ size_t off_S() const { return 0; }
    __host__ __device__ size_t lds_doubles(int M) const {
        size_t o = (size_t)((4 * M + 2 + 1) & ~1) + 32;
        o += (size_t)(tw ? 2 : 1) * (16 * 28 + 64 + 16 * 28) + (size_t)16 * (nRecT + nRecB);
        o += tw ? 2 * 256 : 0;
        return o;
    }
};
__host__ __device__ inline int band_rec_pos(int q) { return (q & 3) * 4 + (q >> 2); }

hipError_t launch_prune_and_setup(const FrameDev *frames_dev, const FrameDev *frames_host, int F, hipStream_t s);
bool prologue_direct_ok(const FrameDev &f);
bool prologue_pair_ok(const FrameDev &f);
hipError_t launch_prologue_direct(const FrameDev *fh, const double *host_up, double *dev_up, int up_doubles, int yin_off, unsigned epoch, hipStream_t s,
                                  const FrameDev *f2 = nullptr, const double *host_up2 = nullptr, double *dev_up2 = nullptr, int up_doubles2 = 0);
hipError_t launch_iteration(const FrameDev *frames_dev, const FrameDev *frames_host, int F, hipStream_t s, int iteration = -1);
hipError_t launch_iteration_timed(const FrameDev *frames_dev, const FrameDev *frames_host, int F, hipStream_t s, hipEvent_t e_start, hipEvent_t e_stop,
                                  hipEvent_t m_start, hipEvent_t m_stop, int iteration = -1);
const char *mstep_kernel_name(const FrameDev *frames_host, int F);
hipError_t launch_estep2(const FrameDev *frames_dev, const FrameDev *frames_host, int F, hipStream_t s, hipEvent_t ev_start = nullptr, hipEvent_t ev_stop = nullptr);
size_t estep2_lds_bytes(int M, int tile_rows);
hipError_t launch_estep_only(const FrameDev *frames_dev, const FrameDev *frames_host, int F, int kind, hipStream_t s);
hipError_t launch_split_setup(const FrameDev *frames_dev, const FrameDev *frames_host, hipStream_t s);
hipError_t launch_split_set_global(const FrameDev *frames_dev, double Nglob, double Sglob, hipStream_t s);
hipError_t launch_split_init_pack(const FrameDev *frames_dev, double *init2, hipStream_t s);
hipError_t launch_split_set_global_dev(const FrameDev *frames_dev, const double *init2, hipStream_t s);
hipError_t launch_split_poll_pack(const FrameDev *frames_dev, double *out2, hipStream_t s);
hipError_t launch_xch_init(const FrameDev *frames_dev, hipStream_t s);
hipError_t launch_split_dmin_xch(const FrameDev *frames_dev, const FrameDev *frames_host, double *xch, int import, hipStream_t s);
hipError_t launch_debug_exp2(const double *x, double *y, int n, hipStream_t s);
hipError_t launch_node_min_dist(const double *X, int N, const double *Y, int M, unsigned long long *out_bits, hipStream_t s);
hipError_t launch_node_min_dist_direct(const double *X, int N, const double *Yhost, int M, unsigned long long *state, unsigned long long *res_host, unsigned epoch, hipStream_t s);
size_t mstep_lds_bytes(int M);
hipError_t launch_mstep_big(const FrameDev *frames_dev, const FrameDev *frames_host, int F, int from_sums, bool f64, hipStream_t s);
size_t mstep_big_scratch_doubles(int M);
hipError_t launch_mstep_pivot_mcu(const FrameDev *frames_dev, const FrameDev *frames_host, int F, int from_sums, bool f64, hipStream_t s);
bool mstep_pivot_mcu_enabled();
bool mstep_mcu_enabled();
hipError_t launch_mstep_chain(const FrameDev *frames_dev, const FrameDev *frames_host, int F, int from_sums, bool f64, hipStream_t s);
hipError_t launch_iter_fused(const FrameDev &fr, const FrameDev &fw, int iteration, hipStream_t s);
size_t iter_fused_lds_bytes(int M);
hipError_t launch_mstep_chain_close(const FrameDev &f, int iteration, hipStream_t s);
void mstep_parity_hint(int iteration);
hipError_t launch_lle_band_debug(const double *Y_dev, int M, double *Hb_dev, hipStream_t s);
bool mstep_chain_enabled();
int mstep_set_dense(int on);
hipError_t launch_mstep_band(const FrameDev *frames_dev, const FrameDev *frames_host, int F, int from_sums, bool f64, hipStream_t s);
size_t band_record_doubles(int M);
size_t mstep_band_lds_bytes(int M);
bool mstep_band_enabled();
int mstep_set_lle_dense(int on);
size_t reg_ws_doubles(int M, int nblk);
int reg_max_nodes();
hipError_t launch_reg(const double *X, int N, int M, double mu, int max_iter, int nblk, double *ws, hipStream_t s);
struct CloudColour { const unsigned char *colour, *occluder; unsigned lo[4], span[4]; int n, rgb; };
size_t cloud_ws_bytes(int P);
hipError_t launch_cloud_bbox(const unsigned short *depth, const unsigned char *mask, int P, int cols, const double cam[4], unsigned *bbox, void *ws, hipStream_t s);
hipError_t launch_cloud_voxels(const unsigned short *depth, const unsigned char *mask, int P, int cols, const double cam[4],
                               const int min_b[3], int mul1, int mul2, float inv_leaf, int nodown, int passes, int n,
                               void *ws, int *total_dev, int cap, double *Xraw, hipStream_t s);
struct CloudViewSrc { const void *data; bool f64; long long stride_point, stride_comp; const unsigned char *select; };
hipError_t launch_view_bbox(const CloudViewSrc &v, int N, unsigned *bbox, void *ws, hipStream_t s);
hipError_t launch_view_voxels(const CloudViewSrc &v, int N, const int min_b[3], int mul1, int mul2, float inv_leaf, int nodown, int passes, int n,
                              void *ws, int *total_dev, int cap, double *Xraw, hipStream_t s);
size_t cloud_fused_ws_bytes(int P);
int cloud_fused_max_points();
bool cloud_fused_ok(int P);
hipError_t launch_cloud_fused(const unsigned short *depth, const unsigned char *mask, int P, int cols, const double cam[4], float inv_leaf, void *ws, void *fws,
                              bool first, bool team, double *Xraw, int cap, unsigned long long *res_pinned, unsigned epoch, hipStream_t s,
                              const double *vis_nodes_pinned = nullptr, int vis_M = 0, unsigned long long *vis_state = nullptr, unsigned long long *vis_out_pinned = nullptr,
                              const CloudColour *colour = nullptr);
hipError_t launch_colour_mask(const CloudColour &colour, int P, unsigned char *mask, unsigned char *hsv, hipStream_t s);
int check_device_image();
hipError_t launch_render(const unsigned char *colour, const unsigned char *occluder, unsigned char *out, const int *prims, int n_prims, int P, int cols,
                         unsigned *corner, hipStream_t s);
int cloud_import_form(const void *src, bool f64, long long stride_point, long long stride_comp);
hipError_t launch_cloud_import(const void *src, bool f64, long long stride_point, long long stride_comp, int N, double *Xraw, hipStream_t s);
struct ImageJob;
hipError_t launch_image_import(const ImageJob &job, hipStream_t s);

}
```

trackdlo_amd/csrc/tdlo_iter_fused.hip:

```cpp
#include "tdlo_mstep_chain_body.h"
#include "tdlo_estep_body.h"
#include <hip/hip_ext.h>
#include <type_traits>

namespace tdlo {

struct FusedLaunch {
    IterState *st_w;
    double *Y_w, *Yout_w;
    void *nodes_w;
    long long *acc_clr;
    int iteration;
    int acc_r;
    int err_r;
};

constexpr size_t kFusedStateBytes = 128;
static_assert(sizeof(IterState) <= kFusedStateBytes, "IterState outgrew its LDS slot");
static size_t fused_estep_bytes(int M) { return (estep_lds_bytes<float, kCB>(M, true) + 15) & ~(size_t)15; }

template <typename T>
__global__ __launch_bounds__(kCB) void k_iter_fused(const FrameDev f0, const FusedLaunch a, const unsigned estep_bytes) {
    constexpr int NCH = 1, EB = kCB;
    constexpr bool VIS = false, SINGLE = true, FUSED = true;
    const FrameDev &f = f0;
    extern __shared__ __attribute__((aligned(16))) char smem[];
    EstepHand<T> h;
    {
        const void *p0 = f.Xs, *p1 = f.st, *p2 = f.chain, *p3 = f.nodes, *p4 = f.Y, *p5 = f.Y0, *p6 = f.aJ, *p7 = f.aYd, *p8 = f.acc, *p9 = f.sync, *p10 = f.ctr;
        asm volatile("" :: "s"(p0), "s"(p1), "s"(p2), "s"(p3), "s"(p4), "s"(p5), "s"(p6), "s"(p7), "s"(p8), "s"(p9), "s"(p10),
                     "s"(f.N0), "s"(f.M), "s"(f.ldx), "s"(f.has_priors), "s"(f.host_epoch), "s"(f.acc_sh[0]), "s"(f.acc_sh[1]), "s"(f.acc_sh[2]),
                     "s"(a.acc_r), "s"(a.err_r), "s"(estep_bytes));
        h.acc_rows = acc_rows_used(f);
        asm volatile("" : "+s"(h.acc_rows));
        h.x = 0; h.y = 0; h.z = 0;
        const auto xs = TDLO_AS_GLOBAL(T, f.Xs);
        const size_t ld = f.ldx;
        const int n = ((int)blockIdx.x * (EB / 64) + (int)(threadIdx.x >> 6)) * 64 + (int)(threadIdx.x & 63);
        if (n < f.N0) { h.x = xs[n]; h.y = xs[ld + n]; h.z = xs[2 * ld + n]; }
        ChainFused z;
        z.iteration = a.iteration; z.err_r = a.err_r;
        z.st_w = a.st_w; z.Y_w = a.Y_w; z.Yout_w = a.Yout_w; z.nodes_w = a.nodes_w; z.acc_clr = a.acc_clr;
        z.stL = (IterState *)(smem + estep_bytes);
        z.nodesL = smem;
        z.go = false;
        mstep_chain_run<T, true, false, false, kAccRows, true, 1>(f, 0, smem + estep_bytes + kFusedStateBytes, a.acc_r, &z);
        if (!z.go) return;
        asm volatile("" :: "s"(__builtin_amdgcn_kernarg_segment_ptr()));
        h.st = z.stL;
        h.acc_buf = a.acc_r == 2 ? 0 : a.acc_r + 1;
        h.err_w = a.err_r ^ 1;
    }
    const EstepHand<T> *const hand = &h;
#include "tdlo_estep_body.inc"
}

size_t iter_fused_lds_bytes(int M) { return fused_estep_bytes(M) + kFusedStateBytes + ChainCarve(M).total * sizeof(double); }

hipError_t launch_iter_fused(const FrameDev &fr, const FrameDev &fw, int iteration, hipStream_t s) {
    const int M = fr.M;
    if (M > kChunk || fr.precision != TDLO_PREC_F32 || fr.vis_branch || fr.eb != kCB || !fr.wide_tile || fr.estep2) return hipErrorInvalidValue;
    const size_t lds = iter_fused_lds_bytes(M);
    if (lds > 64 * 1024) { const hipError_t e = hipFuncSetAttribute((const void *)k_iter_fused<float>, hipFuncAttributeMaxDynamicSharedMemorySize, (int)lds); if (e != hipSuccess) return e; }
    FusedLaunch a;
    a.st_w = fw.st; a.Y_w = fw.Y; a.Yout_w = fw.Yout; a.nodes_w = fw.nodes;
    a.acc_clr = fr.acc + (size_t)((iteration + 2) % 3) * kAccRows * acc_stride(M);
    a.iteration = iteration; a.acc_r = iteration % 3; a.err_r = (iteration + 1) & 1;
    hipLaunchKernelGGL(k_iter_fused<float>, dim3(fr.nblkE), dim3(kCB), lds, s, fr, a, (unsigned)fused_estep_bytes(M));
    return hipGetLastError();
}

}
```

trackdlo_amd/csrc/tdlo_mstep_chain_body.h:

```cpp
#pragma once
#include <type_traits>
#include "tdlo_devcommon.h"
#include "tdlo_lle_dev.h"
#include <atomic>
#include <cstdlib>
#include <hip/hip_ext.h>

namespace tdlo {
namespace {

constexpr int kCB = 256;
typedef double dbl2 __attribute__((ext_vector_type(2)));

__device__ __forceinline__ double swap_add32(double x, double y) {
    const auto lo = __builtin_amdgcn_permlane32_swap((unsigned)__double2loint(x), (unsigned)__double2loint(y), false, false);
    const auto hi = __builtin_amdgcn_permlane32_swap((unsigned)__double2hiint(x), (unsigned)__double2hiint(y), false, false);
    return __hiloint2double((int)hi[0], (int)lo[0]) + __hiloint2double((int)hi[1], (int)lo[1]);
}
__device__ __forceinline__ double swap_add16(double x, double y) {
    const auto lo = __builtin_amdgcn_permlane16_swap((unsigned)__double2loint(x), (unsigned)__double2loint(y), false, false);
    const auto hi = __builtin_amdgcn_permlane16_swap((unsigned)__double2hiint(x), (unsigned)__double2hiint(y), false, false);
    return __hiloint2double((int)hi[0], (int)lo[0]) + __hiloint2double((int)hi[1], (int)lo[1]);
}
template <int CTRL> __device__ __forceinline__ double dpp_f64c(double v) {
    const int lo = __builtin_amdgcn_update_dpp(0, __double2loint(v), CTRL, 0xf, 0xf, false), hi = __builtin_amdgcn_update_dpp(0, __double2hiint(v), CTRL, 0xf, 0xf, false);
    return __hiloint2double(hi, lo);
}
__device__ __forceinline__ double wave_sum4(double a, double b, double c, double d) {
    double z = swap_add16(swap_add32(a, b), swap_add32(c, d));
    z += dpp_f64c<0x128>(z);
    z += dpp_f64c<0x124>(z);
    z += dpp_f64c<0x122>(z);
    z += dpp_f64c<0x121>(z);
    return z;
}

template <int L> __device__ __forceinline__ double row_bcast_f64(double v) {
    const int lo = __builtin_amdgcn_update_dpp(0, __double2loint(v), 0x150 + L, 0xf, 0xf, false);
    const int hi = __builtin_amdgcn_update_dpp(0, __double2hiint(v), 0x150 + L, 0xf, 0xf, false);
    return __hiloint2double(hi, lo);
}

}

constexpr int kSlot = 34;
constexpr int kAhead = 6;
constexpr int kBehind = 9;
constexpr int kDump = 32;
constexpr int kRed = 112;
constexpr int kND = 4;
constexpr int kDirectMax = 21;

struct ChainCarve {
    int nSp, j1, j2, j3, n0, n1, n2, n3, nQ, nSl;
    size_t S, red, dump, slots, total;
    __host__ __device__ explicit ChainCarve(int M) {
        nSp = 4 * M + 2;
        j2 = (M - 1) >> 1; j1 = j2 >> 1; j3 = (j2 + M) >> 1;
        n0 = j1 + 1; n1 = j2 - j1; n2 = j3 - j2 + 1; n3 = M - j3;
        const int a = n0 > n1 ? n0 : n1, b = n2 > n3 ? n2 : n3;
        nQ = a > b ? a : b;
        nSl = kND * nQ;
        size_t o = 0;
        S = o; o += (size_t)((nSp + 1) & ~1);
        red = o; o += kRed;
        dump = o; o += kDump;
        o += (size_t)kSlot * kBehind;
        slots = o; o += (size_t)kSlot * (nSl + kAhead);
        total = o;
    }
};

struct ChainFused {
    int iteration;
    int err_r;
    IterState *st_w;
    double *Y_w, *Yout_w;
    void *nodes_w;
    long long *acc_clr;
    IterState *stL;
    void *nodesL;
    bool go;
};
template <typename T, bool SINGLE, bool XCH, bool TRK = false, int ROWS = kAccRows, bool HINT = false, int FUSE = 0>
__device__ __forceinline__ void mstep_chain_run(const FrameDev &f, int from_sums, char *smem, int par_hint = 0, ChainFused *fz = nullptr) {
    static_assert(FUSE == 0 || (SINGLE && HINT && !XCH && !TRK), "the one-launch iteration: one frame, told its accumulator buffer, no exchange / tracker extras");
    constexpr int MB = kCB;
    IterState *st = f.st;
    const int M = f.M, t = threadIdx.x, lane = t & 63;
    const int wv = __builtin_amdgcn_readfirstlane(t >> 6);
    const int nS = 4 * M + 1;
    const ChainCarve cv(M);
    const int nQ = cv.nQ, nSl = cv.nSl, j1 = cv.j1, j2 = cv.j2, j3 = cv.j3;
    const int padbits = (nQ - cv.n0) | ((nQ - cv.n1) << 4) | ((nQ - cv.n2) << 8) | ((nQ - cv.n3) << 12);
    double *S = (double *)smem + cv.S, *red = (double *)smem + cv.red, *dump = (double *)smem + cv.dump, *slots = (double *)smem + cv.slots;

#ifdef TDLO_CHAIN_STAMPS
#define CSTAMP(i) do { if (t == 0 && (FUSE != 1 || blockIdx.x == 0)) f.dbg[(FUSE == 1 ? 56 : 0) + (i)] = __builtin_amdgcn_s_memtime(); } while (0)
#else
#define CSTAMP(i) do { } while (0)
#endif
    CSTAMP(0);
    if (SINGLE) {
        const void *p0 = f.st, *p1 = f.chain, *p2 = f.nodes, *p3 = f.Y, *p4 = f.Y0, *p5 = f.aJ, *p6 = f.aYd;
        asm volatile("" :: "s"(p0), "s"(p1), "s"(p2), "s"(p3), "s"(p4), "s"(p5), "s"(p6));
    }
    const auto stg = TDLO_AS_GLOBAL(IterState, st);
    const bool err_w = FUSE != 0 && TDLO_AS_GLOBAL(unsigned, f.sync)[kFusedErrWord + (FUSE != 0 ? fz->err_r : 0)] == f.host_epoch;
    const int done = FUSE != 0 ? (stg->done | (err_w ? 1 : 0)) : stg->done;
    const double sigma2 = stg->sigma2;
    int pri = f.has_priors;
    if constexpr (FUSE == 1) asm volatile("" : "+s"(pri));
    const double ctr0 = f.ctr[0], ctr1 = f.ctr[1], ctr2 = f.ctr[2];
    const auto ndg = TDLO_AS_GLOBAL(V4<T>, f.nodes);
    const auto Yg = TDLO_AS_GLOBAL(double, f.Y);
    const auto Y0g = TDLO_AS_GLOBAL(double, f.Y0);
    const bool late_src = TRK && f.late_aJ != nullptr && (from_sums == 1 || f.late_mstep != 0);
    const auto aJg = TDLO_AS_GLOBAL(double, late_src ? f.late_aJ : f.aJ);
    const auto aYg = TDLO_AS_GLOBAL(double, late_src ? f.late_aYd : f.aYd);
    const auto chg = TDLO_AS_GLOBAL(dbl2, f.chain);

    auto slot_dir = [&](int sl) __attribute__((always_inline)) { return (int)(sl >= nQ) + (int)(sl >= 2 * nQ) + (int)(sl >= 3 * nQ); };
    auto slot_info = [&](int sl, int &node, int &li, bool &obs) __attribute__((always_inline)) {
        const int dir = slot_dir(sl), k = sl - dir * nQ;
        const int kk = k - ((padbits >> (4 * dir)) & 15);
        const bool real = kk >= 0;
        int nd, l; bool ob;
        if (dir == 0)      { nd = kk;         l = kk > 0 ? kk : 0;     ob = true; }
        else if (dir == 1) { nd = j2 - 1 - kk; l = nd + 1;             ob = nd != j1; }
        else if (dir == 2) { nd = j2 + kk;    l = kk > 0 ? nd : 0;     ob = nd != j3 && !(kk == 0 && j1 == j2); }
        else               { nd = M - 1 - kk; l = kk > 0 ? nd + 1 : 0; ob = true; }
        node = real ? nd : 0; li = real ? l : 0; obs = real && ob;
    };
    struct SlotQ { dbl2 l[4]; double y[3], y0[3], yp[3], ay[3], aj, w; int node, li; bool obs; };
    auto load_slot = [&](int sl, bool with_pri) __attribute__((always_inline)) {
        SlotQ q;
        slot_info(sl < nSl ? sl : 0, q.node, q.li, q.obs);
        const int lc = q.li > 0 ? q.li : 1, mc = q.node;
#pragma unroll
        for (int i = 0; i < 4; ++i) q.l[i] = chg[4 * (size_t)lc + i];
        q.y[0] = (double)ndg[mc].x; q.y[1] = (double)ndg[mc].y; q.y[2] = (double)ndg[mc].z; q.w = (double)ndg[mc].w;
#pragma unroll
        for (int d = 0; d < 3; ++d) { q.y0[d] = Y0g[d * M + mc]; q.yp[d] = Yg[d * M + mc]; q.ay[d] = (pri && with_pri) ? aYg[d * M + mc] : 0.0; }
        q.aj = (pri && with_pri) ? aJg[mc] : 0.0;
        return q;
    };
    const bool spec_wait = TRK && f.spec_flag != nullptr;
    const int itn = FUSE == 1 ? fz->iteration : stg->it;
    constexpr int kStWords = (int)((sizeof(IterState) + 7) / 8);
    unsigned long long st_word = 0;
    if constexpr (FUSE == 1) st_word = TDLO_AS_GLOBAL(unsigned long long, st)[t < kStWords ? t : kStWords - 1];
    double sq[9];
    SlotQ q0;
    long long fr0[ROWS], fr1[ROWS];
    const int fi0 = t < nS ? t : nS - 1, fi1 = t + MB < nS ? t + MB : nS - 1;
    if constexpr (FUSE == 1) {
        const auto rows = TDLO_AS_GLOBAL(long long, f.acc) + (size_t)par_hint * kAccRows * acc_stride(M);
        const int stride = acc_stride(M);
#pragma unroll
        for (int r = 0; r < ROWS; ++r) fr0[r] = rows[(size_t)r * stride + fi0];
        if (nS > MB) {
#pragma unroll
            for (int r = 0; r < ROWS; ++r) fr1[r] = rows[(size_t)r * stride + fi1];
        } else {
#pragma unroll
            for (int r = 0; r < ROWS; ++r) fr1[r] = 0;
        }
        sq[0] = 0.0;
    } else
    sq[0] = HINT ? acc_read_par<ROWS>(f, t < nS ? t : nS - 1, par_hint) : acc_read_both<ROWS>(f, t < nS ? t : nS - 1, itn);
#pragma unroll
    for (int u = 1; u < 9; ++u) sq[u] = 0.0;
    if constexpr (FUSE == 1) {
        q0 = load_slot(t, true);
    } else if (nS <= MB) {
        q0 = load_slot(t, !spec_wait);
    } else {
        if (from_sums != 1) {
            const auto rows = TDLO_AS_GLOBAL(long long, f.acc) + (size_t)(HINT ? par_hint : (itn & 1)) * kAccRows * acc_stride(M);
            const int stride = acc_stride(M);
            auto more = [&](auto U0c, auto U1c) __attribute__((always_inline)) {
                constexpr int U0 = decltype(U0c)::value, U1 = decltype(U1c)::value;
                long long sa[U1 - U0];
                int ix[U1 - U0];
#pragma unroll
                for (int u = U0; u < U1; ++u) {
                    const int i = t + u * MB;
                    ix[u - U0] = i < nS ? i : nS - 1;
                    long long a = 0;
#pragma unroll
                    for (int r = 0; r < ROWS; ++r) a += rows[(size_t)r * stride + ix[u - U0]];
                    sa[u - U0] = a;
                }
#pragma unroll
                for (int u = U0; u < U1; ++u) sq[u] = ::ldexp((double)sa[u - U0], -acc_shift(f, ix[u - U0]));
            };
            using std::integral_constant;
            switch ((nS + MB - 1) / MB) {
                case 2: if (t + MB < nS) sq[1] = HINT ? acc_read_par<ROWS>(f, t + MB, par_hint) : acc_read_both<ROWS>(f, t + MB, itn); break;
                case 3: more(integral_constant<int, 1>(), integral_constant<int, 3>()); break;
                case 4: more(integral_constant<int, 1>(), integral_constant<int, 4>()); break;
                case 5: more(integral_constant<int, 1>(), integral_constant<int, 5>()); break;
                default:
#pragma unroll
                    for (int u = 1; u < 9; ++u) { const int i = t + u * MB; if (i < nS) sq[u] = HINT ? acc_read_par<ROWS>(f, i, par_hint) : acc_read_both<ROWS>(f, i, itn); }
                    break;
            }
        }
        q0 = load_slot(t, !spec_wait);
    }
    double ss[5] = {0.0, 0.0, 0.0, 0.0, 0.0};
    if (TRK && from_sums == 1) {
        const auto sums = TDLO_AS_GLOBAL(double, f.sums);
#pragma unroll
        for (int u = 0; u < 5; ++u) { const int i = t + u * MB; ss[u] = sums[i < nS ? i : nS - 1]; }
    }
    if (spec_wait) {
        if (f.spec_prev != nullptr) {
            const auto pv = TDLO_AS_GLOBAL(IterState, f.spec_prev);
            if (!(pv->done != 0 && pv->status == 0)) return;
        }
        if (t == 0) {
            const unsigned long long t0 = __builtin_amdgcn_s_memrealtime();
            int go = 0;
            for (;;) {
                const unsigned long long v = __hip_atomic_load(f.spec_flag, __ATOMIC_RELAXED, __HIP_MEMORY_SCOPE_SYSTEM);
                if ((unsigned)(v >> 32) == f.spec_epoch && (v & 3ull) != 0ull) {
                    go = (v & 3ull) == 1ull;
                    __builtin_amdgcn_fence(__ATOMIC_ACQUIRE, "");
                    break;
                }
                if (__builtin_amdgcn_s_memrealtime() - t0 > 200000000ull) break;
                __builtin_amdgcn_s_sleep(4);
            }
            red[31] = go ? 1.0 : 0.0;
        }
        __syncthreads();
        const bool go = red[31] != 0.0;
        __syncthreads();
        if (!go) {
            if (f.late_mstep != 0 && from_sums == 0) acc_clear_other<MB>(f, 1, t);
            return;
        }
    }
    if (spec_wait && pri) {
#pragma unroll
        for (int d = 0; d < 3; ++d) q0.ay[d] = aYg[d * M + q0.node];
        q0.aj = aJg[q0.node];
    }
    double kq[4] = {0.0, 0.0, 0.0, 0.0};
    if (late_src && pri) {
#pragma unroll
        for (int u = 0; u < 4; ++u) { const int i = t + u * MB, ic = i < 4 * M ? i : 4 * M - 1; kq[u] = ic < M ? aJg[ic] : aYg[ic - M]; }
    }
    dbl2 ch0 = dbl2{0.0, 0.0}, ch1 = dbl2{0.0, 0.0};
    double Nc_f = 0.0;
    if constexpr (FUSE == 1) {
        ch0 = chg[0]; ch1 = chg[1]; Nc_f = stg->Nc;
        asm volatile("; TDLO_FUSED_PROLOGUE_REQUESTED" ::: "memory");
        asm volatile("" :: "s"(__builtin_amdgcn_kernarg_segment_ptr()));
        auto fused_sum = [&](const long long (&rw)[ROWS], int i) __attribute__((always_inline)) {
            long long a = 0;
#pragma unroll
            for (int r = 0; r < ROWS; ++r) a += rw[r];
            const int sh = f.acc_sh[0] + (i >= M ? f.acc_sh[1] - f.acc_sh[0] : 0) + (i >= 4 * M ? f.acc_sh[2] - f.acc_sh[1] : 0);
            return ::ldexp((double)a, -sh);
        };
        sq[0] = fused_sum(fr0, fi0);
        if (t + MB < nS) sq[1] = fused_sum(fr1, fi1);
        if (t < kStWords) ((unsigned long long *)fz->stL)[t] = st_word;
    }
    const double pinf0 = FUSE == 1 ? ch0.x : chg[0].x, pinf1 = FUSE == 1 ? ch0.y : chg[0].y;
    const double c2 = f.lambda * sigma2, rc2 = fast_rcp(c2);
    const double cp0 = c2 * (FUSE == 1 ? ch1.x : chg[1].x), cp1 = c2 * (FUSE == 1 ? ch1.y : chg[1].y);
    const double Nc = FUSE == 1 ? Nc_f : stg->Nc;
    const double kc = f.mu / (1.0 - f.mu) * (f.vis_branch ? 1.0 / Nc : (double)M / Nc);
#ifdef TDLO_TIMELINE
    if (t == 0 && itn >= 20 && itn < 28) f.dbg[4 * (itn - 20) + 2] = __builtin_amdgcn_s_memrealtime();
#endif
    if constexpr (FUSE == 1) {
        if (done) {
            fz->go = false;
            if (blockIdx.x != 0) return;
            for (int i = t; i < 3 * M; i += MB) fz->Yout_w[i] = f.Yout[i];
            __syncthreads();
            if (t < 64) {
                constexpr int nst = (int)((sizeof(IterState) + 7) / 8);
                if (lane < nst) ((unsigned long long *)fz->st_w)[lane] = TDLO_AS_GLOBAL(unsigned long long, st)[lane];
                const bool err_new = err_w && stg->done == 0;
                if (err_new && lane == 0) { asm volatile("s_waitcnt vmcnt(0)" ::: "memory"); fz->st_w->status = TDLO_E_NUMERIC; fz->st_w->converged = 0; fz->st_w->done = 1; }
                if (stg->status != 0 || err_new) host_publish_at(f, fz->Yout_w, fz->st_w, lane, false);
            }
            return;
        }
        fz->go = true;
    }
    if (FUSE == 2 && err_w && stg->done == 0) {
        if (t == 0) { st->status = TDLO_E_NUMERIC; st->converged = 0; st->done = 1; }
        if (t < 64) host_publish(f, st, lane, false);
        return;
    }
    if (done) {
        if (XCH && from_sums == 3) xch_post_error(f, st, t);
        if (!XCH && t < 64 && stg->status != 0) host_publish(f, st, lane, false);
        return;
    }
    CSTAMP(1);
    if (HINT && FUSE == 0 && from_sums != 1 && (itn & 1) != par_hint) {
#pragma unroll
        for (int u = 0; u < 9; ++u) { const int i = t + u * MB; if (i < nS) sq[u] = acc_read_both<ROWS>(f, i, itn); }
    }
    if (from_sums != 1) {
        constexpr int nU = FUSE == 1 ? 2 : 9;
#pragma unroll
        for (int u = 0; u < nU; ++u) { const int i = t + u * MB; if (i < nS) S[i] = sq[u]; }
    } else {
        const auto sums = TDLO_AS_GLOBAL(double, f.sums);
        if (TRK) {
#pragma unroll
            for (int u = 0; u < 5; ++u) { const int i = t + u * MB; if (i < nS) S[i] = ss[u]; }
            for (int i = t + 5 * MB; i < nS; i += MB) S[i] = sums[i];
        } else {
            for (int i = t; i < nS; i += MB) S[i] = sums[i];
        }
    }
    if (late_src && pri) {
        double *aJw = (double *)f.aJ, *aYw = (double *)f.aYd;
#pragma unroll
        for (int u = 0; u < 4; ++u) { const int i = t + u * MB; if (i < M) aJw[i] = kq[u]; else if (i < 4 * M) aYw[i - M] = kq[u]; }
        for (int i = t + 4 * MB; i < 4 * M; i += MB) aYw[i - M] = aYg[i - M];
    }
    __syncthreads();
    if (from_sums == 2) {
        acc_clear_other<MB>(f, itn, t);
        for (int i = t; i < nS; i += MB) f.sums[i] = S[i];
        if (t == 0) f.sums[nS] = (double)stg->N;
        return;
    }
    if (XCH && from_sums == 3 && (f.xch_nranks > 1 || f.xch_self)) {
        const int R = f.xch_nranks, me = f.xch_rank, Mc = f.xch_mcap, it = stg->it, par = it & 1;
        const unsigned long long tag = ((unsigned long long)f.xch_epoch << 32) | (unsigned)(it + 1);
        const size_t so = xch_off_sums(R, Mc), sl = 4 * (size_t)Mc + 2;
        for (int i = t; i < nS; i += MB) {
            const double v = S[i];
            for (int q = 0; q < R; ++q) xch_store_f64(xch_ptr(f.xch_inbox[q]) + so + ((size_t)par * R + me) * sl + i, v);
        }
        xch_release();
        __syncthreads();
        if (t < R) xch_store(xch_ptr(f.xch_inbox[t]) + xch_off_flag_sums(R) + par * R + me, tag);
        const xch_word *own = xch_ptr(f.xch_inbox[me]);
        if (t == 0) red[24] = 1.0;
        __syncthreads();
        if (t < R) { const int w_ = xch_wait_sums(own + xch_off_flag_sums(R) + par * R + t, tag); if (w_ != 1) red[24] = w_ == 0 ? 0.0 : -1.0; }
        __syncthreads();
        xch_acquire();
        if (red[24] != 1.0) { if (t == 0) { st->status = red[24] == 0.0 ? TDLO_E_EXCHANGE : TDLO_E_NUMERIC; st->done = 1; st->converged = 0; } return; }
        for (int i = t; i < nS; i += MB) {
            double a = 0;
            for (int r = 0; r < R; ++r) a += xch_load_f64(own + so + ((size_t)par * R + r) * sl + i);
            S[i] = a;
        }
        __syncthreads();
    }
    CSTAMP(2);

    for (int sl = t, r = 0; sl < nSl; sl += MB, ++r) {
        dbl2 *o = (dbl2 *)(slots + (size_t)kSlot * sl);
        const SlotQ q = r == 0 ? q0 : load_slot(sl, true);
        const double p1 = q.obs ? S[q.node] : 0.0;
        const bool idl = q.li == 0;
        o[0] = dbl2{idl ? 1.0 : q.l[0].x, idl ? 0.0 : q.l[0].y}; o[1] = dbl2{idl ? 0.0 : q.l[1].x, idl ? 1.0 : q.l[1].y};
        o[2] = dbl2{idl ? 0.0 : q.l[2].x * rc2, idl ? 0.0 : q.l[2].y * rc2};
        o[3] = dbl2{idl ? 0.0 : q.l[3].x * rc2, q.obs ? p1 + q.aj : 0.0};
#pragma unroll
        for (int d = 0; d < 3; ++d) o[4 + d] = dbl2{q.obs ? S[(1 + d) * M + q.node] + (p1 * (q.y[d] - q.y0[d]) + q.ay[d]) : 0.0, 0.0};
    }
    if (t == 0) { *(int *)(red + 28) = 0; red[26] = 0.0; red[27] = 0.0; }
    if (t >= MB - kAhead) {
        dbl2 *o = (dbl2 *)(slots + (size_t)kSlot * (nSl + (t - (MB - kAhead))));
        o[0] = dbl2{1.0, 0.0}; o[1] = dbl2{0.0, 1.0}; o[2] = dbl2{0.0, 0.0}; o[3] = dbl2{0.0, 0.0}; o[4] = dbl2{0.0, 0.0}; o[5] = dbl2{0.0, 0.0}; o[6] = dbl2{0.0, 0.0};
    }
    __syncthreads();
    CSTAMP(3);

    constexpr int SB = kSlot * 8;
    const unsigned prog_addr = (unsigned)(uintptr_t)(__attribute__((address_space(3))) void *)(red + 28);
    if (wv == 0) {
        const int dir = lane >> 4, hl = lane & 15;
        const bool inner = dir == 1 || dir == 2;
        char *const sb = (char *)slots, *const db = (char *)dump;
        char *ra = sb + (size_t)SB * dir * nQ;
        char *qa = hl == 0 ? ra : db;
        const int qstep = hl == 0 ? SB : 0;
        double a = inner ? 0.0 : pinf0 * rc2, b = 0.0, d = inner ? 0.0 : pinf1 * rc2;
        struct Rec { dbl2 r0, r1, r2, r3; };
        auto fetch = [&](int ahead) __attribute__((always_inline)) {
            Rec r;
            const char *rp = ra + SB * ahead;
            r.r0 = *(const dbl2 *)(rp); r.r1 = *(const dbl2 *)(rp + 16); r.r2 = *(const dbl2 *)(rp + 32); r.r3 = *(const dbl2 *)(rp + 48);
            return r;
        };
        int kdone = 0;
        auto step = [&](const Rec &r, int at) __attribute__((always_inline)) {
            const double f11 = r.r0.x, f12 = r.r0.y, f21 = r.r1.x, f22 = r.r1.y, q11 = r.r2.x, q12 = r.r2.y, q22 = r.r3.x, p = r.r3.y;
            const double t1 = fma(f12, b, f11 * a), t2 = fma(f12, d, f11 * b);
            const double t3 = fma(f22, b, f21 * a), t4 = fma(f22, d, f21 * b);
            const double pa = fma(t2, f12, fma(t1, f11, q11));
            const double pb = fma(t2, f22, fma(t1, f21, q12));
            const double pd = fma(t4, f22, fma(t3, f21, q22));
            const double g = fast_rcp(fma(p, pa, 1.0));
            const double npb = -(p * pb);
            a = pa * g; b = pb * g; d = fma(npb, b, pd);
            *(dbl2 *)(qa + qstep * at + 160) = dbl2{a, b};
            *(dbl2 *)(qa + qstep * at + 176) = dbl2{d, g};
            ++kdone;
            asm volatile("ds_write_b32 %0, %1" :: "v"(prog_addr), "v"(kdone) : "memory");
        };
        int k = 0;
        if (nQ >= 4) {
            Rec rA = fetch(0), rB = fetch(1);
            for (; k + 3 < nQ; k += 4) {
                const Rec rC = fetch(2), rD = fetch(3);
                step(rA, 0); step(rB, 1);
                rA = fetch(4); rB = fetch(5);
                step(rC, 2); step(rD, 3);
                ra += 4 * SB; qa += 4 * qstep;
            }
        }
        for (; k < nQ; ++k) {
            const Rec r = fetch(0);
            step(r, 0);
            ra += SB; qa += qstep;
        }
    } else if (wv == 1) {
        const int dir = lane >> 4, hl = lane & 15;
        const bool wr = hl < 5;
        char *const sb = (char *)slots, *const db = (char *)dump;
        char *ra = sb + (size_t)SB * dir * nQ;
        char *la = wr ? (hl < 3 ? ra + 16 * hl : ra + 112 + 16 * (hl - 3)) : db;
        const int lstep = wr ? SB : 0;
        const char *ba = hl < 3 ? ra + 64 + 16 * hl : (const char *)(red + 26);
        const int bstep = hl < 3 ? SB : 0;
        double m0 = hl == 3 ? 1.0 : 0.0, m1 = hl == 4 ? 1.0 : 0.0;
        const double sgl = hl < 3 ? 1.0 : -1.0;
        double acc0 = 0.0, acc1 = 0.0;
        int have = 0;
        auto wait_for = [&](int need) __attribute__((always_inline)) {
            while (have < need) {
                int v;
                asm volatile("ds_read_b32 %0, %1\n\ts_waitcnt lgkmcnt(0)" : "=v"(v) : "v"(prog_addr) : "memory");
                have = __builtin_amdgcn_readfirstlane(v);
                if (have < need) __builtin_amdgcn_s_sleep(1);
            }
        };
        struct MRec { dbl2 r0, r1, ab; double p, bb, g; };
        auto mfetch = [&](int ahead) __attribute__((always_inline)) {
            MRec r;
            const char *rp = ra + SB * ahead;
            r.r0 = *(const dbl2 *)(rp); r.r1 = *(const dbl2 *)(rp + 16); r.p = *(const double *)(rp + 56); r.ab = *(const dbl2 *)(rp + 160);
            r.bb = *(const double *)(ba + bstep * ahead);
            r.g = *(const double *)(rp + 184);
            return r;
        };
        auto mstep = [&](const MRec &r, int at) __attribute__((always_inline)) {
            const double pm0 = fma(r.r0.y, m1, r.r0.x * m0), pm1 = fma(r.r1.y, m1, r.r1.x * m0);
            const double innov = fma(-r.p, pm0, r.bb);
            const double w = (sgl * r.g) * innov;
            const double h0 = row_bcast_f64<3>(pm0), h1 = row_bcast_f64<4>(pm0);
            acc0 = fma(w, h0, acc0); acc1 = fma(w, h1, acc1);
            m0 = fma(r.ab.x, innov, pm0); m1 = fma(r.ab.y, innov, pm1);
            *(dbl2 *)(la + lstep * at + 112) = dbl2{m0, m1};
        };
        int k = 0;
        for (; k + 3 < nQ; k += 2) {
            wait_for(k + 2);
            const MRec rA = mfetch(0), rB = mfetch(1);
            mstep(rA, 0); mstep(rB, 1);
            ra += 2 * SB; la += 2 * lstep; ba += 2 * bstep;
        }
        for (; k < nQ; ++k) {
            wait_for(k + 1);
            const MRec r = mfetch(0);
            mstep(r, 0);
            ra += SB; la += lstep; ba += bstep;
        }
        if (wr) *(dbl2 *)(red + 32 + 2 * (dir * 5 + hl)) = dbl2{acc0, acc1};
    } else {
        if constexpr (FUSE == 1) {
            if (blockIdx.x == 0) { const int n = kAccRows * acc_stride(M); for (int i = t - 128; i < n; i += MB - 128) fz->acc_clr[i] = 0; }
        } else if constexpr (FUSE == 2) {
        } else
        if (from_sums != 1) acc_clear_other<MB - 128>(f, itn, t - 128);
        if (wv == 2) {
            int have = 0;
            while (have < nQ) {
                int v;
                asm volatile("ds_read_b32 %0, %1\n\ts_waitcnt lgkmcnt(0)" : "=v"(v) : "v"(prog_addr) : "memory");
                have = __builtin_amdgcn_readfirstlane(v);
                if (have < nQ) __builtin_amdgcn_s_sleep(4);
            }
            const int hf = lane >> 5, dO = hf ? 3 : 0, dI = hf ? 2 : 1;
            const double *sO = slots + (size_t)kSlot * (dO * nQ + nQ - 1), *sI = slots + (size_t)kSlot * (dI * nQ + nQ - 1);
            const dbl2 abO = *(const dbl2 *)(sO + 20), abI = *(const dbl2 *)(sI + 20);
            const double Oa = abO.x, Ob = -abO.y, Od = sO[22], pa = abI.x, pb = abI.y, pd = sI[22];
            const double rO = fast_rcp(fma(Oa, Od, -(Ob * Ob)));
            const double ia = Od * rO, ib = -Ob * rO, id = Oa * rO;
            const double La = ia - cp0, Lb = ib, Ld = id - cp1;
            const double n00 = fma(La, pa, fma(Lb, pb, 1.0)), n01 = fma(La, pb, Lb * pd), n10 = fma(Lb, pa, Ld * pb), n11 = fma(Lb, pb, fma(Ld, pd, 1.0));
            const double rn = fast_rcp(fma(n00, n11, -(n01 * n10)));
            const double A00 = n11 * rn, A01 = -n01 * rn, A10 = -n10 * rn, A11 = n00 * rn;
            const double W00 = fma(A00, La, A01 * Lb), W01 = fma(A00, Lb, A01 * Ld), W11 = fma(A10, Lb, A11 * Ld);
            dbl2 *jo = (dbl2 *)((lane & 31) == 0 ? red + 80 + 16 * hf : dump);
            jo[0] = dbl2{ia, ib}; jo[1] = dbl2{id, La}; jo[2] = dbl2{Lb, Ld}; jo[3] = dbl2{A00, A01}; jo[4] = dbl2{A10, A11}; jo[5] = dbl2{W00, W01}; jo[6] = dbl2{W11, 0.0};
        }
    }
    __syncthreads();
    CSTAMP(4);
    for (int sl = t; sl < nSl; sl += MB) {
        const int dir = slot_dir(sl), k = sl - dir * nQ;
        if (k < nQ - 1) {
            double *o = slots + (size_t)kSlot * sl;
            const dbl2 *np = (const dbl2 *)(o + kSlot);
            const double h11 = np[0].x, h12 = np[0].y, h21 = np[1].x, h22 = np[1].y, q11 = np[2].x, q12 = np[2].y, q22 = np[3].x;
            const dbl2 ab = *(const dbl2 *)(o + 20);
            const double a = ab.x, b = ab.y, d = o[22];
            const double t1 = fma(h12, b, h11 * a), t2 = fma(h12, d, h11 * b);
            const double t3 = fma(h22, b, h21 * a), t4 = fma(h22, d, h21 * b);
            const double pa = fma(t2, h12, fma(t1, h11, q11)), pb = fma(t2, h22, fma(t1, h21, q12)), pd = fma(t4, h22, fma(t3, h21, q22));
            const double det = fma(pa, pd, -(pb * pb));
            const double rdet = det > 0.0 ? fast_rcp(det) : 0.0;
            const double ia = pd * rdet, ib = -pb * rdet, id = pa * rdet;
            const double C11 = fma(t1, ia, t3 * ib), C12 = fma(t1, ib, t3 * id), C21 = fma(t2, ia, t4 * ib), C22 = fma(t2, ib, t4 * id);
            const int nq = (dir == 1 || dir == 2) ? 5 : 3;
#pragma unroll
            for (int q = 0; q < 5; ++q) {
                if (q < nq) {
                    dbl2 *mp = (dbl2 *)(o + (q < 3 ? 14 + 2 * q : 22 + 2 * q));
                    const dbl2 mm = *mp;
                    const double pm0 = fma(h12, mm.y, h11 * mm.x), pm1 = fma(h22, mm.y, h21 * mm.x);
                    *mp = dbl2{mm.x - fma(C11, pm0, C12 * pm1), mm.y - fma(C21, pm0, C22 * pm1)};
                }
            }
            *(dbl2 *)(o + 24) = dbl2{C11, C12};
            *(dbl2 *)(o + 26) = dbl2{C21, C22};
        }
    }
    if (wv == 1) {
        const int hf = lane >> 5, hl = lane & 31, dd = hl < 3 ? hl : 2;
        const int dO = hf ? 3 : 0, dI = hf ? 2 : 1;
        double *sO = slots + (size_t)kSlot * (dO * nQ + nQ - 1), *sI = slots + (size_t)kSlot * (dI * nQ + nQ - 1);
        const dbl2 mO = *(const dbl2 *)(sO + 14 + 2 * dd), gI = *(const dbl2 *)(sI + 14 + 2 * dd);
        const dbl2 abI = *(const dbl2 *)(sI + 20);
        const dbl2 *jm = (const dbl2 *)(red + 80 + 16 * hf);
        const dbl2 j0 = jm[0], j1v = jm[1], j2v = jm[2], j3v = jm[3], j4v = jm[4], j5v = jm[5];
        const double W11 = red[80 + 16 * hf + 12];
        const dbl2 Fc0 = *(const dbl2 *)(sI + 28), Fc1 = *(const dbl2 *)(sI + 30);
        const dbl2 aE = *(const dbl2 *)(red + 32 + 2 * (dI * 5 + dd)), aJ0 = *(const dbl2 *)(red + 32 + 2 * (dI * 5 + 3)), aJ1 = *(const dbl2 *)(red + 32 + 2 * (dI * 5 + 4));
        const double m0 = mO.x, m1 = -mO.y;
        const double pa = abI.x, pb = abI.y, pd = sI[22];
        const double F00 = Fc0.x, F10 = Fc0.y, F01 = Fc1.x, F11 = Fc1.y, g0 = gI.x, g1 = gI.y;
        const double ia = j0.x, ib = j0.y, id = j1v.x, La = j1v.y, Lb = j2v.x, Ld = j2v.y, A00 = j3v.x, A01 = j3v.y, A10 = j4v.x, A11 = j4v.y;
        const double W00 = j5v.x, W01 = j5v.y, W10 = j5v.y;
        const double xi0 = fma(ia, m0, ib * m1), xi1 = fma(ib, m0, id * m1);
        const double w0 = fma(A00, xi0, A01 * xi1), w1 = fma(A10, xi0, A11 * xi1);
        const double v0 = w0 - fma(W00, g0, W01 * g1), v1 = w1 - fma(W10, g0, W11 * g1);
        const double WF00 = fma(W00, F00, W01 * F10), WF01 = fma(W00, F01, W01 * F11), WF10 = fma(W10, F00, W11 * F10), WF11 = fma(W10, F01, W11 * F11);
        const double sg = hf ? 1.0 : -1.0;
        double J00 = fma(F00, WF00, F10 * WF10) + aJ0.x, J01 = sg * (fma(F00, WF01, F10 * WF11) + aJ0.y), J11 = fma(F01, WF01, F11 * WF11) + aJ1.y;
        double e0 = fma(F00, v0, F10 * v1) + aE.x, e1 = sg * (fma(F01, v0, F11 * v1) + aE.y);
        J00 = swap_add32(J00, J00); J01 = swap_add32(J01, J01); J11 = swap_add32(J11, J11); e0 = swap_add32(e0, e0); e1 = swap_add32(e1, e1);
        J00 += cp0; J11 += cp1;
        const double rJ = fast_rcp(fma(J00, J11, -(J01 * J01)));
        const double x0 = (J11 * e0 - J01 * e1) * rJ, x1 = (J00 * e1 - J01 * e0) * rJ;
        const double s0 = x0, s1 = sg * x1;
        const double u0 = fma(F00, s0, fma(F01, s1, g0)), u1 = fma(F10, s0, fma(F11, s1, g1));
        const double r0 = xi0 - fma(La, u0, Lb * u1), r1 = xi1 - fma(Lb, u0, Ld * u1);
        const double z0 = fma(A00, r0, A01 * r1), z1 = fma(A10, r0, A11 * r1);
        const double y0 = fma(pa, z0, fma(pb, z1, u0)), y1 = fma(pb, z0, fma(pd, z1, u1));
        wave_lds_sync();
        if (hl < 3) {
            *(dbl2 *)(sI + 14 + 2 * hl) = dbl2{y0, y1};
            *(dbl2 *)(sO + 14 + 2 * hl) = dbl2{y0, -y1};
            if (hf) *(dbl2 *)(red + 72 + 2 * hl) = dbl2{x0, x1};
        }
    }
    __syncthreads();
    CSTAMP(5);
    const bool direct = nQ <= kDirectMax;
    if (direct) {
        if (wv == 0) {
            const int dir = lane >> 4, hl = lane & 15;
            const bool wr = hl < 3, inner = dir == 1 || dir == 2;
            char *const sb = (char *)slots, *const db = (char *)dump;
            const char *ra = sb + (size_t)SB * (dir * nQ + nQ - 1);
            char *la = wr ? (char *)ra + 16 * hl : db;
            const int lstep = wr ? SB : 0;
            dbl2 xs = dbl2{0.0, 0.0};
            if (inner && wr) { xs = *(const dbl2 *)(red + 72 + 2 * hl); if (dir == 1) xs.y = -xs.y; }
            const dbl2 xj = *(const dbl2 *)(la + 112);
            double x0 = xj.x, x1 = xj.y;
            struct BRec { dbl2 e, C0, C1, E0, E1; };
            auto bfetch = [&](int i) __attribute__((always_inline)) {
                BRec r;
                const char *sp = ra - SB * i;
                r.e = *(const dbl2 *)(la - lstep * i + 112); r.C0 = *(const dbl2 *)(sp + 192); r.C1 = *(const dbl2 *)(sp + 208);
                r.E0 = *(const dbl2 *)(sp + 224); r.E1 = *(const dbl2 *)(sp + 240);
                return r;
            };
            auto bstep = [&](const BRec &r, int i) __attribute__((always_inline)) {
                const double e0 = fma(r.E0.x, xs.x, fma(r.E1.x, xs.y, r.e.x)), e1 = fma(r.E0.y, xs.x, fma(r.E1.y, xs.y, r.e.y));
                const double y0 = fma(r.C0.x, x0, fma(r.C0.y, x1, e0)), y1 = fma(r.C1.x, x0, fma(r.C1.y, x1, e1));
                x0 = y0; x1 = y1;
                *(dbl2 *)(la - lstep * i + 112) = dbl2{x0, x1};
            };
            int k = 1;
            BRec rA = bfetch(1), rB = bfetch(2);
            for (; k + 3 < nQ; k += 4) {
                const BRec rC = bfetch(3), rD = bfetch(4);
                bstep(rA, 1); bstep(rB, 2);
                rA = bfetch(5); rB = bfetch(6);
                bstep(rC, 3); bstep(rD, 4);
                ra -= 4 * SB; la -= 4 * lstep;
            }
            const int rem = nQ - k;
            if (rem >= 1) bstep(rA, 1);
            if (rem >= 2) bstep(rB, 2);
            if (rem >= 3) { const BRec r = bfetch(3); bstep(r, 3); }
        }
        __syncthreads();
    } else {
    for (int sl = t; sl < nSl; sl += MB) {
        const int k = sl - slot_dir(sl) * nQ;
        if (k < nQ - 1) {
            double *o = slots + (size_t)kSlot * sl;
            const int r4 = (nQ - 1 - k) & 3, j = r4 ? r4 : 4;
            const double *top = o + (size_t)kSlot * (j - 1);
            dbl2 c0 = *(const dbl2 *)(top + 24), c1 = *(const dbl2 *)(top + 26);
            const int dir = slot_dir(sl);
            const bool inner = dir == 1 || dir == 2;
            dbl2 xs[3];
#pragma unroll
            for (int q = 0; q < 3; ++q) { xs[q] = inner ? *(const dbl2 *)(red + 72 + 2 * q) : dbl2{0.0, 0.0}; if (dir == 1) xs[q].y = -xs[q].y; }
            auto e_of = [&](const double *s, dbl2 (&e)[3]) __attribute__((always_inline)) {
#pragma unroll
                for (int q = 0; q < 3; ++q) e[q] = *(const dbl2 *)(s + 14 + 2 * q);
                if (inner) {
                    const dbl2 E0 = *(const dbl2 *)(s + 28), E1 = *(const dbl2 *)(s + 30);
#pragma unroll
                    for (int q = 0; q < 3; ++q) e[q] = dbl2{fma(E0.x, xs[q].x, fma(E1.x, xs[q].y, e[q].x)), fma(E0.y, xs[q].x, fma(E1.y, xs[q].y, e[q].y))};
                }
            };
            dbl2 ev[3];
            e_of(top, ev);
            for (int i = j - 2; i >= 0; --i) {
                const double *s = o + (size_t)kSlot * i;
                const dbl2 d0 = *(const dbl2 *)(s + 24), d1 = *(const dbl2 *)(s + 26);
                dbl2 es[3];
                e_of(s, es);
#pragma unroll
                for (int q = 0; q < 3; ++q) ev[q] = dbl2{fma(d0.x, ev[q].x, fma(d0.y, ev[q].y, es[q].x)), fma(d1.x, ev[q].x, fma(d1.y, ev[q].y, es[q].y))};
                const dbl2 n0 = dbl2{fma(d0.x, c0.x, d0.y * c1.x), fma(d0.x, c0.y, d0.y * c1.y)};
                const dbl2 n1 = dbl2{fma(d1.x, c0.x, d1.y * c1.x), fma(d1.x, c0.y, d1.y * c1.y)};
                c0 = n0; c1 = n1;
            }
            *(dbl2 *)(o + 0) = c0; *(dbl2 *)(o + 2) = c1;
#pragma unroll
            for (int q = 0; q < 3; ++q) *(dbl2 *)(o + 8 + 2 * q) = ev[q];
        }
    }
    __syncthreads();
    if (wv == 0) {
        const int dir = lane >> 4, hl = lane & 15;
        const bool wr = hl < 3;
        char *const sb = (char *)slots, *const db = (char *)dump;
        char *ra = sb + (size_t)SB * (dir * nQ + nQ - 1);
        char *la = wr ? ra + 16 * hl : db;
        const int lstep = wr ? SB : 0;
        const dbl2 xj = *(const dbl2 *)(la + 112);
        double xs0 = xj.x, xs1 = xj.y;
        const int na = (nQ - 1) >> 2;
        struct ARec { dbl2 e, C0, C1; };
        auto afetch = [&](int i) __attribute__((always_inline)) {
            ARec r;
            r.e = *(const dbl2 *)(la - 4 * lstep * i + 64); r.C0 = *(const dbl2 *)(ra - 4 * SB * i); r.C1 = *(const dbl2 *)(ra - 4 * SB * i + 16);
            return r;
        };
        auto astep = [&](const ARec &r, int i) __attribute__((always_inline)) {
            const double y0 = fma(r.C0.x, xs0, fma(r.C0.y, xs1, r.e.x));
            const double y1 = fma(r.C1.x, xs0, fma(r.C1.y, xs1, r.e.y));
            xs0 = y0; xs1 = y1;
            *(dbl2 *)(la - 4 * lstep * i + 112) = dbl2{xs0, xs1};
        };
        int i = 0;
        ARec rA = afetch(1), rB = afetch(2);
        for (; i + 1 < na; i += 2) {
            astep(rA, 1); astep(rB, 2);
            ra -= 8 * SB; la -= 8 * lstep;
            rA = afetch(1); rB = afetch(2);
        }
        if (i < na) astep(rA, 1);
    }
    __syncthreads();
    }
    CSTAMP(6);

    V4<T> *nodes_w = (V4<T> *)f.nodes;
    double s_np = 0, s_dr = 0, s_pd = 0, s_cr = 0;
    for (int sl = t, r = 0; sl < nSl; sl += MB, ++r) {
        const SlotQ q = r == 0 ? q0 : load_slot(sl, true);
        if (!q.obs) continue;
        const int m = q.node;
        const double *o = slots + (size_t)kSlot * sl;
        const double p1 = S[m];
        const int ks = sl - slot_dir(sl) * nQ, r4 = (nQ - 1 - ks) & 3;
        double Vd[3];
        if (direct || r4 == 0) {
#pragma unroll
            for (int d = 0; d < 3; ++d) Vd[d] = o[14 + 2 * d];
        } else {
            const double *an = o + (size_t)kSlot * r4;
            const dbl2 c0 = *(const dbl2 *)(o + 0);
#pragma unroll
            for (int d = 0; d < 3; ++d) { const dbl2 xa = *(const dbl2 *)(an + 14 + 2 * d); Vd[d] = fma(c0.x, xa.x, fma(c0.y, xa.y, o[8 + 2 * d])); }
        }
        double Td[3], cr2 = 0, dr = 0, pd2 = 0;
#pragma unroll
        for (int d = 0; d < 3; ++d) {
            Td[d] = q.y0[d] + Vd[d];
            const double del = Td[d] - q.y[d], ex = q.yp[d] - Td[d];
            dr = fma(del, S[(1 + d) * M + m], dr); pd2 = fma(del, del, pd2); cr2 = fma(ex, ex, cr2);
        }
        s_np += p1; s_dr += dr; s_pd += p1 * pd2; s_cr += ::sqrt(cr2);
        V4<T> w; w.x = (T)Td[0]; w.y = (T)Td[1]; w.z = (T)Td[2]; w.w = (T)q.w;
        if constexpr (FUSE == 1) {
            ((V4<T> *)fz->nodesL)[m] = w;
            if (blockIdx.x == 0) {
                ((V4<T> *)fz->nodes_w)[m] = w;
                f.dminbits[m] = ~0ull;
#pragma unroll
                for (int d = 0; d < 3; ++d) { fz->Y_w[d * M + m] = Td[d]; fz->Yout_w[d * M + m] = Td[d] + (d == 0 ? ctr0 : (d == 1 ? ctr1 : ctr2)); }
            }
        } else {
        nodes_w[m] = w;
        f.dminbits[m] = ~0ull;
#pragma unroll
        for (int d = 0; d < 3; ++d) { f.Y[d * M + m] = Td[d]; f.Yout[d * M + m] = Td[d] + (d == 0 ? ctr0 : (d == 1 ? ctr1 : ctr2)); }
        }
    }
    {
        const double tot = wave_sum4(s_np, s_dr, s_pd, s_cr);
        const int row = lane >> 4, which = ((row & 1) << 1) | (row >> 1);
        double *dst = (lane & 15) == 0 ? red + 4 * wv + which : dump;
        *dst = tot;
    }
    __syncthreads();
    CSTAMP(7);
    IterState *const sto = FUSE == 1 ? fz->stL : st;
    int pub = 0;
    if (t == 0) {
        const double t_np = ((red[0] + red[4]) + red[8]) + red[12], t_dr = ((red[1] + red[5]) + red[9]) + red[13];
        const double t_pd = ((red[2] + red[6]) + red[10]) + red[14], t_cr = ((red[3] + red[7]) + red[11]) + red[15];
        const double new_sigma2 = (S[4 * M] - 2.0 * t_dr + t_pd) * fast_rcp(t_np * 3.0);
        const double crit = t_cr / (double)M;
        const int it = itn + 1;
        sto->it = it; sto->crit = crit; sto->Np = t_np;
        const bool finite_ok = (new_sigma2 == new_sigma2) && (fabs(new_sigma2) < 1e300) && (new_sigma2 > 0) && (crit == crit);
        sto->sigma2 = new_sigma2;
        if (finite_ok) {
            const double tp = 2.0 * M_PI * new_sigma2, rtp = ::sqrt(tp);
            sto->k2 = -1.4426950408889634 * 0.5 * fast_rcp(new_sigma2);
            sto->c_norm = tp * rtp * kc;
            sto->rwin32 = f.win_e32 * 1.3862943611198906 * new_sigma2; sto->rwin64 = f.win_e64 * 1.3862943611198906 * new_sigma2;
            sto->sh_boost = FUSE == 1 ? 0 : acc_boost(f, new_sigma2);
        } else { sto->status = TDLO_E_NUMERIC; sto->done = 1; sto->converged = 0; pub = 1; }
        if (crit < f.tol) { sto->done = 1; pub = 1; }
        else if (it >= f.max_iter) { sto->converged = 0; sto->done = 1; pub = 1; }
        if (it == f.host_report_it) pub = 1;
#ifdef TDLO_TIMELINE
        if (itn >= 20 && itn < 28) f.dbg[4 * (itn - 20) + 3] = __builtin_amdgcn_s_memrealtime();
#endif
    }
    if constexpr (FUSE == 1) {
        __syncthreads();
        fz->go = fz->stL->done == 0;
        if (blockIdx.x == 0 && t < 64) {
            constexpr int nst = (int)((sizeof(IterState) + 7) / 8);
            if (lane < nst) ((unsigned long long *)fz->st_w)[lane] = ((const unsigned long long *)fz->stL)[lane];
            if (__builtin_amdgcn_readfirstlane(pub)) host_publish_at(f, fz->Yout_w, fz->st_w, lane, true);
        }
        return;
    }
    if (!XCH && t < 64 && __builtin_amdgcn_readfirstlane(pub)) host_publish(f, st, lane, true);
    if (TRK && f.lle_next != nullptr) {
        if (t == 0) red[30] = (st->done != 0 && st->status == 0) ? 1.0 : 0.0;
        __syncthreads();
        if (red[30] != 0.0 && M <= 256) lle_band_device<MB>(f.Yout, M, f.lle_next, slots, t);
    }
#undef CSTAMP
}

}
```

Baseline: 85880 EM iterations/s.

## Add wave-0-only fused iteration variant to cut block barriers in M-step chain

Adds a k_iter_fused_w0 kernel variant, used when the slot count fits in one wave. In it the M-step chain runs its slot setup and final reductions on wave 0 with wave-level syncs and readlane reductions instead of block-wide __syncthreads and LDS reductions. The E-step accumulator clearing is moved to the idle waves during the M-step, and the E-step body skips its initial barrier and per-wave clear through a FRONT flag. The goal is less barrier and LDS-reduction overhead on each fused iteration. The cost is more template specialisation and correctness now depends on the cross-wave clear ordering being right.

Result: faster. 88920 EM iterations/s, median of 6 (+3.5%).

```diff
diff --git a/trackdlo_amd/csrc/tdlo_api.cpp b/trackdlo_amd/csrc/tdlo_api.cpp
--- a/trackdlo_amd/csrc/tdlo_api.cpp
+++ b/trackdlo_amd/csrc/tdlo_api.cpp
@@ -244,6 +244,8 @@
     int estep_wide_min = getenv("TDLO_ESTEP_WIDE") ? (atoi(getenv("TDLO_ESTEP_WIDE")) > 0 ? atoi(getenv("TDLO_ESTEP_WIDE")) : (1 << 30)) : kEstepWideMin;
     int fused_iter_mode = getenv("TDLO_FUSED_ITER") ? (atoi(getenv("TDLO_FUSED_ITER")) != 0 ? 1 : 0) : -1;
     long long fused_calls = 0;
+    bool fused_w0_on = !(getenv("TDLO_FUSED_W0") && atoi(getenv("TDLO_FUSED_W0")) == 0);
+    long long fused_w0_calls = 0;
     long long estep2_frames = 0;
     bool timing = false;
     EnqueuePool *pool = nullptr;
@@ -808,6 +810,7 @@
     bool ahead = false;
     bool use_mbox = false;
     bool fused_mode = false;
+    bool fused_w0_seen = false;
     bool late_async = false;
     bool lle_next = false;
     hipStream_t s = nullptr;
@@ -1072,7 +1075,11 @@
         if (fused_mode) {
             const int k = enqueued - 1;
             if (k == 0) TDLO_RET(launch_estep_only(fdp, c->fh.data(), 1, 0, s));
-            if (k + 1 < p->max_iter) TDLO_RET(launch_iter_fused(fused_copy(k), fused_copy(k + 1), k, s));
+            if (k + 1 < p->max_iter) {
+                bool ran_w0 = false;
+                TDLO_RET(launch_iter_fused(fused_copy(k), fused_copy(k + 1), k, c->fused_w0_on, s, &ran_w0));
+                if (ran_w0 && !fused_w0_seen) { fused_w0_seen = true; ++c->fused_w0_calls; }
+            }
             else TDLO_RET(launch_mstep_chain_close(fused_copy(k), k, s));
             continue;
         }
@@ -3129,7 +3136,8 @@
 long long tdlo_debug_band_retries(tdlo_ctx *c) { return c ? c->band_retries : -1; }
 
 long long tdlo_debug_route_count(tdlo_ctx *c, int which) {
-    if (!c || which < 0 || which > 23) return -1;
+    if (!c || which < 0 || which > 24) return -1;
+    if (which == 24) return c->fused_w0_calls;
     if (which >= 22) return c->vis_route[which - 22];
     if (which == 21) return c->voxel_view_calls;
     if (which >= 19) return c->render_route[which - 19];
diff --git a/trackdlo_amd/csrc/tdlo_estep_body.h b/trackdlo_amd/csrc/tdlo_estep_body.h
--- a/trackdlo_amd/csrc/tdlo_estep_body.h
+++ b/trackdlo_amd/csrc/tdlo_estep_body.h
@@ -6,13 +6,37 @@
 
 namespace tdlo {
 
-template <typename T> struct EstepHand {
+template <typename T, bool FRONT = false> struct EstepHand {
+    static constexpr bool kFront = FRONT;
     T x, y, z;
     const IterState *st;
     int acc_buf;
     int err_w;
     int acc_rows;
 };
+
+template <typename T> struct EstepCarve {
+    V4<T> *nodesL;
+    V4<T> *pts;
+    T *lvL;
+    T *pbase;
+    double *scratch;
+};
+template <typename T, int NWE> __device__ __forceinline__ EstepCarve<T> estep_carve(char *smem, int M, int rows) {
+    EstepCarve<T> c;
+    c.nodesL = (V4<T> *)smem;
+    c.pts = c.nodesL + M;
+    c.lvL = (T *)(c.pts + NWE * kPtsStride);
+    c.pbase = c.lvL + ((M + 3) & ~3);
+    c.scratch = (double *)(c.pbase + (((size_t)NWE * rows * kPStride + 7) & ~(size_t)3));
+    return c;
+}
+__device__ __forceinline__ long long *estep_accL(double *scratch, int M, int wave, bool per_wave) {
+    return (long long *)(scratch + 16) + (per_wave ? (size_t)wave * M * 4 : (size_t)0);
+}
+template <typename T, int EB> __device__ __forceinline__ long long *estep_single_accL(char *smem, int M, int wave) {
+    return estep_accL(estep_carve<T, EB / 64>(smem, M, M < kChunk ? M : kChunk).scratch, M, wave, true);
+}
 
 template <typename T, int EB> static size_t estep_lds_bytes(int M, bool single) {
     const int rt = (M <= kChunk && single) ? kChunk : tile_rows<T>(M <= kChunk ? 1 : 2);
diff --git a/trackdlo_amd/csrc/tdlo_estep_body.inc b/trackdlo_amd/csrc/tdlo_estep_body.inc
--- a/trackdlo_amd/csrc/tdlo_estep_body.inc
+++ b/trackdlo_amd/csrc/tdlo_estep_body.inc
@@ -1,4 +1,5 @@
     constexpr int NWE = EB / 64;
+    constexpr bool FRONT = std::remove_cv_t<std::remove_pointer_t<decltype(hand)>>::kFront;
 #ifdef TDLO_ESTEP_STAMPS
     if (threadIdx.x == 0) atomicMin(&f.dbg[32], (unsigned long long)__builtin_amdgcn_s_memrealtime());
 #endif
@@ -27,11 +28,11 @@
     constexpr int RS = (RT / TR) * TR;
     const int rows = M < RT ? M : RT;
     V4<T> *nodesL = (V4<T> *)smem;
-    V4<T> *pts = nodesL + M;
-    T *lvL = (T *)(pts + NWE * kPtsStride);
-    T *pbase = lvL + ((M + 3) & ~3);
+    V4<T> *pts = FRONT ? estep_carve<T, NWE>(smem, M, rows).pts : nodesL + M;
+    T *lvL = FRONT ? estep_carve<T, NWE>(smem, M, rows).lvL : (T *)(pts + NWE * kPtsStride);
+    T *pbase = FRONT ? estep_carve<T, NWE>(smem, M, rows).pbase : lvL + ((M + 3) & ~3);
     T *pb = pbase + (size_t)wave * rows * kPStride;
-    double *scratch = (double *)(pbase + (((size_t)NWE * rows * kPStride + 7) & ~(size_t)3));
+    double *scratch = FRONT ? estep_carve<T, NWE>(smem, M, rows).scratch : (double *)(pbase + (((size_t)NWE * rows * kPStride + 7) & ~(size_t)3));
 
     const auto nodes = TDLO_AS_CONST(V4<T>, f.nodes);
     const auto xs = TDLO_AS_GLOBAL(T, f.Xs);
@@ -50,7 +51,7 @@
     int N; T k2, cn;
     if constexpr (FUSED) { N = hand->st->N; k2 = (T)hand->st->k2; cn = (T)hand->st->c_norm; }
     else if constexpr (EARLY) { N = stg->N; k2 = (T)stg->k2; cn = (T)stg->c_norm; }
-    const int shb_e = FUSED ? hand->st->sh_boost : (EARLY ? stg->sh_boost : 0);
+    const int shb_e = FRONT ? 0 : (FUSED ? hand->st->sh_boost : (EARLY ? stg->sh_boost : 0));
     const double rwin_e = FUSED ? hand->st->rwin32 : (EARLY ? stg->rwin32 : 0.0);
     const int par_e = FUSED ? hand->acc_buf : (it0 & 1);
     const auto qg = TDLO_AS_GLOBAL(V4<T>, f.nodes);
@@ -111,7 +112,7 @@
             lvL[m] = (T)(-f.k_vis * d * 1.4426950408889634 - ::log2(tot));
         }
     }
-    __syncthreads();
+    if constexpr (!FRONT) __syncthreads();
     ESTAMP(1);
     EPHASE(0);
 
@@ -121,9 +122,9 @@
     const double limP = f.acc_lim[0], limR = f.acc_lim[1] * acc_scale(-shb), limQ = f.acc_lim[2] * acc_scale(-2 * shb);
     const double limQn = acc_scale(51 - (f.acc_sh[2] + 2 * shb));
     bool acc_ok = true;
-    long long *accL = (long long *)(scratch + 16) + (NCH == 1 ? (size_t)wave * M * 4 : (size_t)0);
+    long long *accL = FRONT ? estep_accL(scratch, M, wave, true) : (long long *)(scratch + 16) + (NCH == 1 ? (size_t)wave * M * 4 : (size_t)0);
     if (NCH == 1) {
-        for (int i = lane; i < M * 4; i += 64) accL[i] = 0;
+        if constexpr (!FRONT) for (int i = lane; i < M * 4; i += 64) accL[i] = 0;
     } else {
         for (int i = tid; i < M * 4; i += EB) accL[i] = 0;
         __syncthreads();
diff --git a/trackdlo_amd/csrc/tdlo_internal.h b/trackdlo_amd/csrc/tdlo_internal.h
--- a/trackdlo_amd/csrc/tdlo_internal.h
+++ b/trackdlo_amd/csrc/tdlo_internal.h
@@ -175,7 +175,7 @@
 bool mstep_pivot_mcu_enabled();
 bool mstep_mcu_enabled();
 hipError_t launch_mstep_chain(const FrameDev *frames_dev, const FrameDev *frames_host, int F, int from_sums, bool f64, hipStream_t s);
-hipError_t launch_iter_fused(const FrameDev &fr, const FrameDev &fw, int iteration, hipStream_t s);
+hipError_t launch_iter_fused(const FrameDev &fr, const FrameDev &fw, int iteration, bool w0, hipStream_t s, bool *ran_w0);
 size_t iter_fused_lds_bytes(int M);
 hipError_t launch_mstep_chain_close(const FrameDev &f, int iteration, hipStream_t s);
 void mstep_parity_hint(int iteration);
diff --git a/trackdlo_amd/csrc/tdlo_iter_fused.hip b/trackdlo_amd/csrc/tdlo_iter_fused.hip
--- a/trackdlo_amd/csrc/tdlo_iter_fused.hip
+++ b/trackdlo_amd/csrc/tdlo_iter_fused.hip
@@ -55,18 +55,72 @@
 #include "tdlo_estep_body.inc"
 }
 
+template <typename T>
+__global__ __launch_bounds__(kCB) void k_iter_fused_w0(const FrameDev f0, const FusedLaunch a, const unsigned estep_bytes) {
+    constexpr int NCH = 1, EB = kCB;
+    constexpr bool VIS = false, SINGLE = true, FUSED = true;
+    const FrameDev &f = f0;
+    extern __shared__ __attribute__((aligned(16))) char smem[];
+    EstepHand<T, true> h;
+    {
+        const void *p0 = f.Xs, *p1 = f.st, *p2 = f.chain, *p3 = f.nodes, *p4 = f.Y, *p5 = f.Y0, *p6 = f.aJ, *p7 = f.aYd, *p8 = f.acc, *p9 = f.sync, *p10 = f.ctr;
+        asm volatile("" :: "s"(p0), "s"(p1), "s"(p2), "s"(p3), "s"(p4), "s"(p5), "s"(p6), "s"(p7), "s"(p8), "s"(p9), "s"(p10),
+                     "s"(f.N0), "s"(f.M), "s"(f.ldx), "s"(f.has_priors), "s"(f.host_epoch), "s"(f.acc_sh[0]), "s"(f.acc_sh[1]), "s"(f.acc_sh[2]),
+                     "s"(a.acc_r), "s"(a.err_r), "s"(estep_bytes));
+        h.acc_rows = acc_rows_used(f);
+        asm volatile("" : "+s"(h.acc_rows));
+        h.x = 0; h.y = 0; h.z = 0;
+        const auto xs = TDLO_AS_GLOBAL(T, f.Xs);
+        const size_t ld = f.ldx;
+        const int n = ((int)blockIdx.x * (EB / 64) + (int)(threadIdx.x >> 6)) * 64 + (int)(threadIdx.x & 63);
+        if (n < f.N0) { h.x = xs[n]; h.y = xs[ld + n]; h.z = xs[2 * ld + n]; }
+        ChainFused z;
+        z.iteration = a.iteration; z.err_r = a.err_r;
+        z.st_w = a.st_w; z.Y_w = a.Y_w; z.Yout_w = a.Yout_w; z.nodes_w = a.nodes_w; z.acc_clr = a.acc_clr;
+        z.stL = (IterState *)(smem + estep_bytes);
+        z.nodesL = smem;
+        z.go = false;
+        mstep_chain_run<T, true, false, false, kAccRows, true, 3>(f, 0, smem + estep_bytes + kFusedStateBytes, a.acc_r, &z);
+        if (!z.go) return;
+        {
+            const int wv = __builtin_amdgcn_readfirstlane((int)(threadIdx.x >> 6));
+            if (wv != 0) {
+                long long *const own = estep_single_accL<T, EB>(smem, f.M, wv);
+                for (int i = (int)(threadIdx.x & 63); i < f.M * 4; i += 64) own[i] = 0;
+            }
+            if (wv == 3) {
+                long long *const first = estep_single_accL<T, EB>(smem, f.M, 0);
+                for (int i = (int)(threadIdx.x & 63); i < f.M * 4; i += 64) first[i] = 0;
+            }
+        }
+        mstep_chain_w0_close(f, &z);
+        if (!z.go) return;
+        asm volatile("" :: "s"(__builtin_amdgcn_kernarg_segment_ptr()));
+        h.st = z.stL;
+        h.acc_buf = a.acc_r == 2 ? 0 : a.acc_r + 1;
+        h.err_w = a.err_r ^ 1;
+    }
+    const EstepHand<T, true> *const hand = &h;
+#include "tdlo_estep_body.inc"
+}
+
 size_t iter_fused_lds_bytes(int M) { return fused_estep_bytes(M) + kFusedStateBytes + ChainCarve(M).total * sizeof(double); }
 
-hipError_t launch_iter_fused(const FrameDev &fr, const FrameDev &fw, int iteration, hipStream_t s) {
+static bool iter_fused_w0_fits(int M) { return ChainCarve(M).nSl <= 64; }
+
+hipError_t launch_iter_fused(const FrameDev &fr, const FrameDev &fw, int iteration, bool w0, hipStream_t s, bool *ran_w0) {
     const int M = fr.M;
     if (M > kChunk || fr.precision != TDLO_PREC_F32 || fr.vis_branch || fr.eb != kCB || !fr.wide_tile || fr.estep2) return hipErrorInvalidValue;
     const size_t lds = iter_fused_lds_bytes(M);
-    if (lds > 64 * 1024) { const hipError_t e = hipFuncSetAttribute((const void *)k_iter_fused<float>, hipFuncAttributeMaxDynamicSharedMemorySize, (int)lds); if (e != hipSuccess) return e; }
+    const bool take_w0 = w0 && iter_fused_w0_fits(M);
+    const auto kern = !take_w0 ? k_iter_fused<float> : k_iter_fused_w0<float>;
+    if (lds > 64 * 1024) { const hipError_t e = hipFuncSetAttribute((const void *)kern, hipFuncAttributeMaxDynamicSharedMemorySize, (int)lds); if (e != hipSuccess) return e; }
     FusedLaunch a;
     a.st_w = fw.st; a.Y_w = fw.Y; a.Yout_w = fw.Yout; a.nodes_w = fw.nodes;
     a.acc_clr = fr.acc + (size_t)((iteration + 2) % 3) * kAccRows * acc_stride(M);
     a.iteration = iteration; a.acc_r = iteration % 3; a.err_r = (iteration + 1) & 1;
-    hipLaunchKernelGGL(k_iter_fused<float>, dim3(fr.nblkE), dim3(kCB), lds, s, fr, a, (unsigned)fused_estep_bytes(M));
+    hipLaunchKernelGGL(kern, dim3(fr.nblkE), dim3(kCB), lds, s, fr, a, (unsigned)fused_estep_bytes(M));
+    if (ran_w0) *ran_w0 = take_w0;
     return hipGetLastError();
 }
 
diff --git a/trackdlo_amd/csrc/tdlo_mstep_chain_body.h b/trackdlo_amd/csrc/tdlo_mstep_chain_body.h
--- a/trackdlo_amd/csrc/tdlo_mstep_chain_body.h
+++ b/trackdlo_amd/csrc/tdlo_mstep_chain_body.h
@@ -81,11 +81,14 @@
     IterState *stL;
     void *nodesL;
     bool go;
+    int pub;
 };
 template <typename T, bool SINGLE, bool XCH, bool TRK = false, int ROWS = kAccRows, bool HINT = false, int FUSE = 0>
 __device__ __forceinline__ void mstep_chain_run(const FrameDev &f, int from_sums, char *smem, int par_hint = 0, ChainFused *fz = nullptr) {
     static_assert(FUSE == 0 || (SINGLE && HINT && !XCH && !TRK), "the one-launch iteration: one frame, told its accumulator buffer, no exchange / tracker extras");
     constexpr int MB = kCB;
+    constexpr bool F1 = FUSE == 1 || FUSE == 3;
+    constexpr bool W0 = FUSE == 3;
     IterState *st = f.st;
     const int M = f.M, t = threadIdx.x, lane = t & 63;
     const int wv = __builtin_amdgcn_readfirstlane(t >> 6);
@@ -96,7 +99,7 @@
     double *S = (double *)smem + cv.S, *red = (double *)smem + cv.red, *dump = (double *)smem + cv.dump, *slots = (double *)smem + cv.slots;
 
 #ifdef TDLO_CHAIN_STAMPS
-#define CSTAMP(i) do { if (t == 0 && (FUSE != 1 || blockIdx.x == 0)) f.dbg[(FUSE == 1 ? 56 : 0) + (i)] = __builtin_amdgcn_s_memtime(); } while (0)
+#define CSTAMP(i) do { if (t == 0 && (!F1 || blockIdx.x == 0)) f.dbg[(F1 ? 56 : 0) + (i)] = __builtin_amdgcn_s_memtime(); } while (0)
 #else
 #define CSTAMP(i) do { } while (0)
 #endif
@@ -110,7 +113,7 @@
     const int done = FUSE != 0 ? (stg->done | (err_w ? 1 : 0)) : stg->done;
     const double sigma2 = stg->sigma2;
     int pri = f.has_priors;
-    if constexpr (FUSE == 1) asm volatile("" : "+s"(pri));
+    if constexpr (F1) asm volatile("" : "+s"(pri));
     const double ctr0 = f.ctr[0], ctr1 = f.ctr[1], ctr2 = f.ctr[2];
     const auto ndg = TDLO_AS_GLOBAL(V4<T>, f.nodes);
     const auto Yg = TDLO_AS_GLOBAL(double, f.Y);
@@ -146,20 +149,20 @@
         return q;
     };
     const bool spec_wait = TRK && f.spec_flag != nullptr;
-    const int itn = FUSE == 1 ? fz->iteration : stg->it;
+    const int itn = F1 ? fz->iteration : stg->it;
     constexpr int kStWords = (int)((sizeof(IterState) + 7) / 8);
     unsigned long long st_word = 0;
-    if constexpr (FUSE == 1) st_word = TDLO_AS_GLOBAL(unsigned long long, st)[t < kStWords ? t : kStWords - 1];
+    if constexpr (F1) st_word = TDLO_AS_GLOBAL(unsigned long long, st)[t < kStWords ? t : kStWords - 1];
     double sq[9];
     SlotQ q0;
     long long fr0[ROWS], fr1[ROWS];
     const int fi0 = t < nS ? t : nS - 1, fi1 = t + MB < nS ? t + MB : nS - 1;
-    if constexpr (FUSE == 1) {
+    if constexpr (F1) {
         const auto rows = TDLO_AS_GLOBAL(long long, f.acc) + (size_t)par_hint * kAccRows * acc_stride(M);
         const int stride = acc_stride(M);
 #pragma unroll
         for (int r = 0; r < ROWS; ++r) fr0[r] = rows[(size_t)r * stride + fi0];
-        if (nS > MB) {
+        if (!W0 && nS > MB) {
 #pragma unroll
             for (int r = 0; r < ROWS; ++r) fr1[r] = rows[(size_t)r * stride + fi1];
         } else {
@@ -171,7 +174,7 @@
     sq[0] = HINT ? acc_read_par<ROWS>(f, t < nS ? t : nS - 1, par_hint) : acc_read_both<ROWS>(f, t < nS ? t : nS - 1, itn);
 #pragma unroll
     for (int u = 1; u < 9; ++u) sq[u] = 0.0;
-    if constexpr (FUSE == 1) {
+    if constexpr (F1) {
         q0 = load_slot(t, true);
     } else if (nS <= MB) {
         q0 = load_slot(t, !spec_wait);
@@ -255,7 +258,8 @@
     }
     dbl2 ch0 = dbl2{0.0, 0.0}, ch1 = dbl2{0.0, 0.0};
     double Nc_f = 0.0;
-    if constexpr (FUSE == 1) {
+    double w_p1 = 0.0, w_r[3] = {0.0, 0.0, 0.0};
+    if constexpr (F1) {
         ch0 = chg[0]; ch1 = chg[1]; Nc_f = stg->Nc;
         asm volatile("; TDLO_FUSED_PROLOGUE_REQUESTED" ::: "memory");
         asm volatile("" :: "s"(__builtin_amdgcn_kernarg_segment_ptr()));
@@ -267,18 +271,18 @@
             return ::ldexp((double)a, -sh);
         };
         sq[0] = fused_sum(fr0, fi0);
-        if (t + MB < nS) sq[1] = fused_sum(fr1, fi1);
+        if (!W0 && t + MB < nS) sq[1] = fused_sum(fr1, fi1);
         if (t < kStWords) ((unsigned long long *)fz->stL)[t] = st_word;
     }
-    const double pinf0 = FUSE == 1 ? ch0.x : chg[0].x, pinf1 = FUSE == 1 ? ch0.y : chg[0].y;
+    const double pinf0 = F1 ? ch0.x : chg[0].x, pinf1 = F1 ? ch0.y : chg[0].y;
     const double c2 = f.lambda * sigma2, rc2 = fast_rcp(c2);
-    const double cp0 = c2 * (FUSE == 1 ? ch1.x : chg[1].x), cp1 = c2 * (FUSE == 1 ? ch1.y : chg[1].y);
-    const double Nc = FUSE == 1 ? Nc_f : stg->Nc;
+    const double cp0 = c2 * (F1 ? ch1.x : chg[1].x), cp1 = c2 * (F1 ? ch1.y : chg[1].y);
+    const double Nc = F1 ? Nc_f : stg->Nc;
     const double kc = f.mu / (1.0 - f.mu) * (f.vis_branch ? 1.0 / Nc : (double)M / Nc);
 #ifdef TDLO_TIMELINE
     if (t == 0 && itn >= 20 && itn < 28) f.dbg[4 * (itn - 20) + 2] = __builtin_amdgcn_s_memrealtime();
 #endif
-    if constexpr (FUSE == 1) {
+    if constexpr (F1) {
         if (done) {
             fz->go = false;
             if (blockIdx.x != 0) return;
@@ -310,8 +314,9 @@
 #pragma unroll
         for (int u = 0; u < 9; ++u) { const int i = t + u * MB; if (i < nS) sq[u] = acc_read_both<ROWS>(f, i, itn); }
     }
+    if constexpr (W0) *(int *)(t == 0 ? red + 28 : dump) = 0;
     if (from_sums != 1) {
-        constexpr int nU = FUSE == 1 ? 2 : 9;
+        constexpr int nU = F1 ? 2 : 9;
 #pragma unroll
         for (int u = 0; u < nU; ++u) { const int i = t + u * MB; if (i < nS) S[i] = sq[u]; }
     } else {
@@ -367,20 +372,22 @@
     for (int sl = t, r = 0; sl < nSl; sl += MB, ++r) {
         dbl2 *o = (dbl2 *)(slots + (size_t)kSlot * sl);
         const SlotQ q = r == 0 ? q0 : load_slot(sl, true);
-        const double p1 = q.obs ? S[q.node] : 0.0;
+        if constexpr (W0) { w_p1 = S[q.node]; w_r[0] = S[M + q.node]; w_r[1] = S[2 * M + q.node]; w_r[2] = S[3 * M + q.node]; }
+        const double p1 = q.obs ? (W0 ? w_p1 : S[q.node]) : 0.0;
         const bool idl = q.li == 0;
         o[0] = dbl2{idl ? 1.0 : q.l[0].x, idl ? 0.0 : q.l[0].y}; o[1] = dbl2{idl ? 0.0 : q.l[1].x, idl ? 1.0 : q.l[1].y};
         o[2] = dbl2{idl ? 0.0 : q.l[2].x * rc2, idl ? 0.0 : q.l[2].y * rc2};
         o[3] = dbl2{idl ? 0.0 : q.l[3].x * rc2, q.obs ? p1 + q.aj : 0.0};
 #pragma unroll
-        for (int d = 0; d < 3; ++d) o[4 + d] = dbl2{q.obs ? S[(1 + d) * M + q.node] + (p1 * (q.y[d] - q.y0[d]) + q.ay[d]) : 0.0, 0.0};
-    }
-    if (t == 0) { *(int *)(red + 28) = 0; red[26] = 0.0; red[27] = 0.0; }
-    if (t >= MB - kAhead) {
-        dbl2 *o = (dbl2 *)(slots + (size_t)kSlot * (nSl + (t - (MB - kAhead))));
+        for (int d = 0; d < 3; ++d) o[4 + d] = dbl2{q.obs ? (W0 ? w_r[d] : S[(1 + d) * M + q.node]) + (p1 * (q.y[d] - q.y0[d]) + q.ay[d]) : 0.0, 0.0};
+    }
+    constexpr int LW = W0 ? 64 : MB;
+    if (t == 0) { if constexpr (!W0) *(int *)(red + 28) = 0; red[26] = 0.0; red[27] = 0.0; }
+    if (t >= LW - kAhead && (!W0 || t < LW)) {
+        dbl2 *o = (dbl2 *)(slots + (size_t)kSlot * (nSl + (t - (LW - kAhead))));
         o[0] = dbl2{1.0, 0.0}; o[1] = dbl2{0.0, 1.0}; o[2] = dbl2{0.0, 0.0}; o[3] = dbl2{0.0, 0.0}; o[4] = dbl2{0.0, 0.0}; o[5] = dbl2{0.0, 0.0}; o[6] = dbl2{0.0, 0.0};
     }
-    __syncthreads();
+    if constexpr (W0) wave_lds_sync(); else __syncthreads();
     CSTAMP(3);
 
     constexpr int SB = kSlot * 8;
@@ -486,7 +493,7 @@
         }
         if (wr) *(dbl2 *)(red + 32 + 2 * (dir * 5 + hl)) = dbl2{acc0, acc1};
     } else {
-        if constexpr (FUSE == 1) {
+        if constexpr (F1) {
             if (blockIdx.x == 0) { const int n = kAccRows * acc_stride(M); for (int i = t - 128; i < n; i += MB - 128) fz->acc_clr[i] = 0; }
         } else if constexpr (FUSE == 2) {
         } else
@@ -586,7 +593,7 @@
     }
     __syncthreads();
     CSTAMP(5);
-    const bool direct = nQ <= kDirectMax;
+    const bool direct = W0 || nQ <= kDirectMax;
     if (direct) {
         if (wv == 0) {
             const int dir = lane >> 4, hl = lane & 15;
@@ -711,7 +718,7 @@
         if (!q.obs) continue;
         const int m = q.node;
         const double *o = slots + (size_t)kSlot * sl;
-        const double p1 = S[m];
+        const double p1 = W0 ? w_p1 : S[m];
         const int ks = sl - slot_dir(sl) * nQ, r4 = (nQ - 1 - ks) & 3;
         double Vd[3];
         if (direct || r4 == 0) {
@@ -728,11 +735,11 @@
         for (int d = 0; d < 3; ++d) {
             Td[d] = q.y0[d] + Vd[d];
             const double del = Td[d] - q.y[d], ex = q.yp[d] - Td[d];
-            dr = fma(del, S[(1 + d) * M + m], dr); pd2 = fma(del, del, pd2); cr2 = fma(ex, ex, cr2);
+            dr = fma(del, W0 ? w_r[d] : S[(1 + d) * M + m], dr); pd2 = fma(del, del, pd2); cr2 = fma(ex, ex, cr2);
         }
         s_np += p1; s_dr += dr; s_pd += p1 * pd2; s_cr += ::sqrt(cr2);
         V4<T> w; w.x = (T)Td[0]; w.y = (T)Td[1]; w.z = (T)Td[2]; w.w = (T)q.w;
-        if constexpr (FUSE == 1) {
+        if constexpr (F1) {
             ((V4<T> *)fz->nodesL)[m] = w;
             if (blockIdx.x == 0) {
                 ((V4<T> *)fz->nodes_w)[m] = w;
@@ -747,19 +754,25 @@
         for (int d = 0; d < 3; ++d) { f.Y[d * M + m] = Td[d]; f.Yout[d * M + m] = Td[d] + (d == 0 ? ctr0 : (d == 1 ? ctr1 : ctr2)); }
         }
     }
-    {
+    if constexpr (W0) {
+        const double tot = wave_sum4(s_np, s_dr, s_pd, s_cr);
+        auto lane_f64 = [&](double v, int src) __attribute__((always_inline)) {
+            return __hiloint2double(__builtin_amdgcn_readlane(__double2hiint(v), src), __builtin_amdgcn_readlane(__double2loint(v), src));
+        };
+        s_np = tot; s_pd = lane_f64(tot, 16); s_dr = lane_f64(tot, 32); s_cr = lane_f64(tot, 48);
+    } else {
         const double tot = wave_sum4(s_np, s_dr, s_pd, s_cr);
         const int row = lane >> 4, which = ((row & 1) << 1) | (row >> 1);
         double *dst = (lane & 15) == 0 ? red + 4 * wv + which : dump;
         *dst = tot;
     }
-    __syncthreads();
+    if constexpr (!W0) __syncthreads();
     CSTAMP(7);
-    IterState *const sto = FUSE == 1 ? fz->stL : st;
+    IterState *const sto = F1 ? fz->stL : st;
     int pub = 0;
     if (t == 0) {
-        const double t_np = ((red[0] + red[4]) + red[8]) + red[12], t_dr = ((red[1] + red[5]) + red[9]) + red[13];
-        const double t_pd = ((red[2] + red[6]) + red[10]) + red[14], t_cr = ((red[3] + red[7]) + red[11]) + red[15];
+        const double t_np = W0 ? ((s_np + 0.0) + 0.0) + 0.0 : ((red[0] + red[4]) + red[8]) + red[12], t_dr = W0 ? ((s_dr + 0.0) + 0.0) + 0.0 : ((red[1] + red[5]) + red[9]) + red[13];
+        const double t_pd = W0 ? ((s_pd + 0.0) + 0.0) + 0.0 : ((red[2] + red[6]) + red[10]) + red[14], t_cr = W0 ? ((s_cr + 0.0) + 0.0) + 0.0 : ((red[3] + red[7]) + red[11]) + red[15];
         const double new_sigma2 = (S[4 * M] - 2.0 * t_dr + t_pd) * fast_rcp(t_np * 3.0);
         const double crit = t_cr / (double)M;
         const int it = itn + 1;
@@ -771,7 +784,7 @@
             sto->k2 = -1.4426950408889634 * 0.5 * fast_rcp(new_sigma2);
             sto->c_norm = tp * rtp * kc;
             sto->rwin32 = f.win_e32 * 1.3862943611198906 * new_sigma2; sto->rwin64 = f.win_e64 * 1.3862943611198906 * new_sigma2;
-            sto->sh_boost = FUSE == 1 ? 0 : acc_boost(f, new_sigma2);
+            sto->sh_boost = F1 ? 0 : acc_boost(f, new_sigma2);
         } else { sto->status = TDLO_E_NUMERIC; sto->done = 1; sto->converged = 0; pub = 1; }
         if (crit < f.tol) { sto->done = 1; pub = 1; }
         else if (it >= f.max_iter) { sto->converged = 0; sto->done = 1; pub = 1; }
@@ -780,7 +793,8 @@
         if (itn >= 20 && itn < 28) f.dbg[4 * (itn - 20) + 3] = __builtin_amdgcn_s_memrealtime();
 #endif
     }
-    if constexpr (FUSE == 1) {
+    if constexpr (W0) { fz->pub = pub; return; }
+    if constexpr (F1) {
         __syncthreads();
         fz->go = fz->stL->done == 0;
         if (blockIdx.x == 0 && t < 64) {
@@ -799,4 +813,15 @@
 #undef CSTAMP
 }
 
+__device__ __forceinline__ void mstep_chain_w0_close(const FrameDev &f, ChainFused *fz) {
+    const int t = threadIdx.x, lane = t & 63;
+    __syncthreads();
+    fz->go = fz->stL->done == 0;
+    if (blockIdx.x == 0 && t < 64) {
+        constexpr int nst = (int)((sizeof(IterState) + 7) / 8);
+        if (lane < nst) ((unsigned long long *)fz->st_w)[lane] = ((const unsigned long long *)fz->stL)[lane];
+        if (__builtin_amdgcn_readfirstlane(fz->pub)) host_publish_at(f, fz->Yout_w, fz->st_w, lane, true);
+    }
 }
+
+}
```
